# NethermindEth/zinc

Measured on AMD Instinct MI355X. Metric: Zip commit+open MCoeffs/s at 2^24 witness, higher is better.
Workload: dtype i64

## Files before the change

### include/zip_hip.h

```cpp
#ifndef ZIP_HIP_H
#define ZIP_HIP_H

#include <stddef.h>
#include <stdint.h>

#ifdef __cplusplus
extern "C" {
#endif

#define ZIP_HIP_ABI_VERSION 3

#define ZIP_OK 0
#define ZIP_ERR_INVALID_PARAM (-1)
#define ZIP_ERR_SHAPE (-2)
#define ZIP_ERR_HIP (-3)
#define ZIP_ERR_NO_DEVICE (-4)
#define ZIP_ERR_UNSUPPORTED (-5)
#define ZIP_ERR_ALLOC (-6)
#define ZIP_ERR_NULL (-7)

typedef enum { ZIP_MEM_HOST = 0, ZIP_MEM_DEVICE = 1 } zip_mem_kind;

typedef struct zip_ctx zip_ctx;
typedef struct zip_commitment zip_commitment;
// ... 35 lines not shown
int32_t zip_commit(zip_ctx *ctx, const int64_t *evals, size_t n_evals, zip_mem_kind evals_kind,
                   int32_t with_merkle, uint8_t *roots_out, zip_commitment **out);
void zip_commitment_free(zip_commitment *c);

int32_t zip_ctx_set_speculation(zip_ctx *ctx, int32_t on);

int32_t zip_commit_hinted(zip_ctx *ctx, const int64_t *evals, size_t n_evals, zip_mem_kind evals_kind,
                          const uint32_t *cols, uint32_t n_cols, uint8_t *roots_out, zip_commitment **out);

int32_t zip_commitment_device_ptrs(zip_commitment *c, uint64_t **rows, uint8_t **layers, uint8_t **roots);
int32_t zip_commit_download(zip_commitment *c, uint64_t *rows_out, uint8_t *layers_out, uint8_t *roots_out);
int32_t zip_commitment_upload(zip_ctx *ctx, const uint64_t *rows, const uint8_t *layers, const uint8_t *roots,
                              zip_commitment **out);


int32_t zip_open_testing(zip_ctx *ctx, const int64_t *evals, zip_mem_kind evals_kind, const int64_t *coeffs,
                         uint64_t *uprime_out, zip_mem_kind out_kind);
int32_t zip_open_columns(zip_commitment *c, const uint32_t *cols, uint32_t n_cols, uint8_t *wire_out,
                         zip_mem_kind out_kind);
int32_t zip_open_eval(zip_ctx *ctx, const int64_t *evals, zip_mem_kind evals_kind, const uint64_t *q0_mont,
                      const zip_field *field, uint64_t *row_out, zip_mem_kind out_kind);
size_t zip_proof_len(const zip_ctx *ctx, uint32_t n_cols, uint32_t field_limbs);
int32_t zip_open(zip_commitment *c, const int64_t *evals, zip_mem_kind evals_kind, const int64_t *coeffs,
                 const uint32_t *cols, uint32_t n_cols, const uint64_t *q0_mont, const zip_field *field,
                 uint8_t *proof_out, zip_mem_kind out_kind);

int32_t zip_open_shard(zip_commitment *c, const int64_t *evals_d, const int64_t *coeffs, const uint32_t *cols, uint32_t n_cols,
                       const uint64_t *q0_mont, const zip_field *field, uint64_t *uprime_part_d, uint64_t *row_part_d,
                       uint8_t *wire_d);

int32_t zip_commit_open(zip_ctx *ctx, const int64_t *evals, size_t n_evals, zip_mem_kind evals_kind, const int64_t *coeffs,
                        const uint32_t *cols, uint32_t n_cols, const uint64_t *q0_mont, const zip_field *field,
                        uint8_t *roots_out, uint8_t *proof_out, zip_mem_kind out_kind, zip_commitment **out);

typedef struct zip_job zip_job;
int32_t zip_commit_open_begin(zip_ctx *ctx, const int64_t *evals_d, size_t n_evals, const int64_t *coeffs,
                              const uint32_t *cols, uint32_t n_cols, const uint64_t *q0_mont, const zip_field *field,
                              uint8_t *proof_out_d, zip_job **job);
int32_t zip_job_wait(zip_job *job, uint8_t *roots_out);

typedef struct zip_batch zip_batch;
int32_t zip_batch_commit(zip_ctx *ctx, const int64_t *evals, size_t n_evals, uint32_t n_polys, zip_mem_kind evals_kind,
                         uint8_t *roots_out, zip_batch **out);
uint32_t zip_batch_size(const zip_batch *b);
void zip_batch_free(zip_batch *b);
int32_t zip_batch_member(zip_batch *b, uint32_t index, zip_commitment **out);
int32_t zip_batch_open_eval(zip_batch *b, const uint64_t *q0_mont, const zip_field *field, uint64_t *rows_out,
                            zip_mem_kind out_kind);
int32_t zip_batch_open(zip_batch *b, const int64_t *coeffs, const uint32_t *cols, uint32_t n_cols, const uint64_t *q0_mont,
                       const zip_field *field, uint8_t *proofs_out, zip_mem_kind out_kind);

typedef int32_t (*zip_proof_sink)(void *user, const uint8_t *bytes, size_t len);
int32_t zip_open_stream(zip_commitment *c, const int64_t *evals, zip_mem_kind evals_kind, const int64_t *coeffs,
                        const uint32_t *cols, uint32_t n_cols, const uint64_t *q0_mont, const zip_field *field,
                        zip_proof_sink sink, void *user, size_t chunk_bytes);

typedef enum {
    ZIP_VERIFY_ACCEPT = 0,
    ZIP_VERIFY_PROXIMITY_TESTING = 1,
    ZIP_VERIFY_EVAL_CONSISTENCY = 2,
    ZIP_VERIFY_PROXIMITY_Q0 = 3,
    ZIP_VERIFY_MERKLE = 4,
    ZIP_VERIFY_MALFORMED = 5,
    ZIP_VERIFY_OVERFLOW = 6
} zip_verify_verdict;
typedef struct {
    int32_t verdict;
    uint32_t column;
    uint32_t bad_merkle_paths;
    uint32_t malformed_paths;
} zip_verify_report;
int32_t zip_verify(zip_ctx *ctx, const uint8_t *roots, const uint8_t *proof, zip_mem_kind proof_kind, size_t proof_len,
                   const int64_t *coeffs, const uint32_t *cols, uint32_t n_cols, const uint64_t *q0_mont,
                   const uint64_t *q1_mont, const uint64_t *eval_mont, const zip_field *field,
                   zip_verify_report *report);

typedef struct zip_sumcheck zip_sumcheck;
typedef struct {
    uint32_t n_terms;
    uint32_t term_mask[8];
    uint64_t coeff[8][8];
} zip_sumcheck_comb;
int32_t zip_sumcheck_init(int32_t device, const uint64_t *const *mles, zip_mem_kind kind, uint32_t n_mles,
                          uint32_t num_vars, uint32_t degree, const zip_sumcheck_comb *comb, const zip_field *field,
                          zip_sumcheck **out);
int32_t zip_sumcheck_round(zip_sumcheck *s, const uint64_t *r_prev, uint64_t *evaluations_out);
int32_t zip_sumcheck_round_begin(zip_sumcheck *s, const uint64_t *r_prev);
int32_t zip_sumcheck_round_end(zip_sumcheck *s, uint64_t *evaluations_out);
const char *zip_sumcheck_last_error(const zip_sumcheck *s);
void zip_sumcheck_free(zip_sumcheck *s);

typedef struct {
    uint64_t st[25];
    uint8_t buf[136];
    uint32_t buflen;
} zip_keccak_state;

int32_t zip_sumcheck_prove(zip_sumcheck *s, zip_keccak_state *transcript, uint64_t *msgs_out, uint64_t *randomness_out);
void zip_sumcheck_launch_counts(uint64_t *round_kernel_rounds, uint64_t *tail_kernel_launches);

typedef struct zip_ccs zip_ccs;
typedef struct {
    uint32_t n_rows, n_cols;
    const uint32_t *row_ptr, *col_idx;
    const int64_t *values;
} zip_sparse_matrix;
typedef enum { ZIP_CCS_Z_FIELD = 0, ZIP_CCS_MZ = 1, ZIP_CCS_EQ = 2, ZIP_CCS_SECOND = 3 } zip_ccs_table_kind;
int32_t zip_ccs_create(int32_t device, const zip_sparse_matrix *matrices, uint32_t t, uint32_t s, const zip_field *field,
                       zip_ccs **out);
void zip_ccs_free(zip_ccs *c);
const char *zip_ccs_last_error(const zip_ccs *c);
int32_t zip_ccs_set_z(zip_ccs *c, const int64_t *z, size_t z_len, zip_mem_kind kind);
int32_t zip_ccs_eq_table(zip_ccs *c, const uint64_t *r, uint32_t slot);
int32_t zip_ccs_second_table(zip_ccs *c, const uint64_t *r_x, const uint64_t *gamma, uint64_t *v_s_out);
int32_t zip_ccs_eval_matrices(zip_ccs *c, const uint64_t *r_x, const uint64_t *r_y, uint64_t *v_xy_out);
int32_t zip_ccs_table(zip_ccs *c, zip_ccs_table_kind which, uint32_t index, const uint64_t **table_dev);
int32_t zip_ccs_download(zip_ccs *c, zip_ccs_table_kind which, uint32_t index, uint64_t *out);

int32_t zip_field_map_int256(zip_ctx *ctx, const uint64_t *values, uint32_t n, const zip_field *field, uint64_t *out);

int32_t zip_mle_eval(zip_ctx *ctx, const int64_t *evals, zip_mem_kind evals_kind, const uint64_t *q0_mont,
                     const uint64_t *q1_mont, const zip_field *field, uint64_t *value_out);
int32_t zip_commitment_mle_eval(zip_commitment *c, const uint64_t *q0_mont, const uint64_t *q1_mont,
                                const zip_field *field, uint64_t *value_out);

int32_t zip_sum_partials(zip_ctx *ctx, const uint64_t *uparts, const uint64_t *fparts, uint32_t n_parts,
                         const zip_field *field, uint64_t *uprime_out, uint64_t *row_out);

typedef struct zip_mctx zip_mctx;
int32_t zip_mctx_create(const zip_params *params, int32_t n_devices, const int32_t *devices, zip_mctx **out);
void zip_mctx_destroy(zip_mctx *m);
const char *zip_mctx_last_error(const zip_mctx *m);
uint32_t zip_mctx_shards(const zip_mctx *m);
zip_ctx *zip_mctx_shard_ctx(zip_mctx *m, uint32_t shard);
int32_t zip_mctx_set_witness(zip_mctx *m, const int64_t *evals, size_t n_evals);
int32_t zip_mctx_commit_open(zip_mctx *m, const int64_t *evals, const int64_t *coeffs, const uint32_t *cols,
                             uint32_t n_cols, const uint64_t *q0_mont, const zip_field *field, uint8_t *roots_out,
                             uint8_t *proof_out);
int32_t zip_mctx_shard_openings(zip_mctx *m, uint32_t shard, uint8_t **ptr, size_t *bytes, uint32_t *row_begin,
                                uint32_t *row_count);
int32_t zip_mctx_ends(zip_mctx *m, uint8_t **ptr, size_t *u_bytes, size_t *row_bytes);
int32_t zip_mctx_roots(zip_mctx *m, uint32_t shard, uint8_t **ptr);
const char *zip_mctx_roots_path(const zip_mctx *m);

int32_t zip_merkle_trees(int32_t device, const uint64_t *leaves, uint32_t leaf_limbs, uint32_t depth,
                         uint32_t num_trees, zip_mem_kind kind, uint8_t *layers_out);

typedef struct {
    const char *name;
    uint32_t launches;
    float total_ms;
} zip_kernel_time;
int32_t zip_ctx_set_profiling(zip_ctx *ctx, int32_t on);
int32_t zip_ctx_commit_clock(zip_ctx *ctx, double *mhz_out);
int32_t zip_ctx_profile_read(zip_ctx *ctx, zip_kernel_time *out, uint32_t cap);

#ifdef __cplusplus
}
#endif
#endif
```

### zinc_amd/cabi.py

```python
import ctypes as C
import os

import numpy as np

_PKG = os.path.dirname(os.path.abspath(__file__))
LIB_PATH = os.environ.get("ZIP_HIP_LIB_PATH") or os.path.join(_PKG, "lib", "libzip_hip.so")

ZIP_OK = 0
ZIP_ERR_INVALID_PARAM = -1
ZIP_ERR_SHAPE = -2
ZIP_ERR_HIP = -3
ZIP_ERR_NO_DEVICE = -4
ZIP_ERR_UNSUPPORTED = -5
ZIP_ERR_ALLOC = -6
ZIP_ERR_NULL = -7
MEM_HOST, MEM_DEVICE = 0, 1

EXPORTED_SYMBOLS = (
    "zip_abi_version", "zip_strerror", "zip_device_count", "zip_release_cached_memory", "zip_host_register", "zip_host_unregister", "zip_ctx_create", "zip_ctx_destroy",
    "zip_ctx_last_error", "zip_ctx_synchronize", "zip_ctx_stream", "zip_ctx_set_speculation", "zip_commit", "zip_commit_hinted", "zip_commit_open", "zip_commit_open_begin", "zip_job_wait", "zip_commitment_free",
    "zip_commitment_device_ptrs", "zip_commit_download", "zip_commitment_upload", "zip_open_testing",
    "zip_open_columns", "zip_open_eval", "zip_proof_len", "zip_open", "zip_open_shard", "zip_sum_partials", "zip_merkle_trees",
    "zip_ctx_set_profiling", "zip_ctx_profile_read", "zip_ctx_commit_clock",
    "zip_mctx_create", "zip_mctx_destroy", "zip_mctx_last_error", "zip_mctx_shards", "zip_mctx_shard_ctx", "zip_mctx_set_witness",
    "zip_mctx_commit_open", "zip_mctx_shard_openings", "zip_mctx_ends", "zip_mctx_roots", "zip_mctx_roots_path", "zip_verify", "zip_mle_eval", "zip_commitment_mle_eval", "zip_field_map_int256",
    "zip_open_stream", "zip_sumcheck_init", "zip_sumcheck_round", "zip_sumcheck_round_begin", "zip_sumcheck_round_end", "zip_sumcheck_last_error", "zip_sumcheck_free",
    "zip_sumcheck_prove", "zip_sumcheck_launch_counts",
    "zip_ccs_create", "zip_ccs_free", "zip_ccs_last_error", "zip_ccs_set_z", "zip_ccs_eq_table",
    "zip_ccs_second_table", "zip_ccs_table", "zip_ccs_download", "zip_ccs_eval_matrices",
    "zip_batch_commit", "zip_batch_size", "zip_batch_free", "zip_batch_member", "zip_batch_open_eval", "zip_batch_open",
)


class Job:

    def __init__(self, ctx, handle, keep):
        self._ctx, self._h, self._keep = ctx, handle, keep

    def wait(self, want_roots=False):
        assert self._h is not None, "job already waited for"
        roots = np.zeros((self._ctx.rows_local, 32), dtype=np.uint8) if want_roots else None
        h, self._h = self._h, None
        rc = lib().zip_job_wait(h, roots.ctypes.data if roots is not None else None)
        self._keep = None
        self._ctx._check(rc, "zip_job_wait")
        return roots

    def close(self):
        if self._h is not None:
            h, self._h = self._h, None
            try:
                lib().zip_job_wait(h, None)
            finally:
                self._keep = None

    def __enter__(self):
        return self

    def __exit__(self, *exc):
        self.close()

    def __del__(self):
        try:
            self.close()
        except Exception:
            pass


class ZipError(RuntimeError):
    def __init__(self, code, what, detail=""):
        self.code = code
        super().__init__(f"{what}: {strerror(code)} ({code})" + (f": {detail}" if detail else ""))


class ZipParams(C.Structure):
    _fields_ = [
        ("num_vars", C.c_uint32), ("row_len", C.c_uint32), ("num_rows", C.c_uint32),
        ("codeword_len", C.c_uint32), ("rep", C.c_uint32),
        ("n_limbs", C.c_uint32), ("k_limbs", C.c_uint32), ("m_limbs", C.c_uint32),
        ("perm1", C.POINTER(C.c_uint32)), ("perm2", C.POINTER(C.c_uint32)),
        ("device", C.c_int32), ("row_begin", C.c_uint32), ("row_count", C.c_uint32),
    ]


class ZipField(C.Structure):
    _fields_ = [("limbs", C.c_uint32), ("modulus", C.c_uint64 * 8)]


class VerifyReport(C.Structure):
    _fields_ = [("verdict", C.c_int32), ("column", C.c_uint32), ("bad_merkle_paths", C.c_uint32),
                ("malformed_paths", C.c_uint32)]


VERIFY_ACCEPT, VERIFY_PROXIMITY_TESTING, VERIFY_EVAL_CONSISTENCY, VERIFY_PROXIMITY_Q0 = 0, 1, 2, 3
VERIFY_MERKLE, VERIFY_MALFORMED, VERIFY_OVERFLOW = 4, 5, 6


class SumcheckComb(C.Structure):
    _fields_ = [("n_terms", C.c_uint32), ("term_mask", C.c_uint32 * 8), ("coeff", (C.c_uint64 * 8) * 8)]


class KeccakState(C.Structure):
    _fields_ = [("st", C.c_uint64 * 25), ("buf", C.c_uint8 * 136), ("buflen", C.c_uint32)]

    @classmethod
    def make(cls, st=None, buf=b""):
        k = cls()
        if st is not None:
            for i, w in enumerate(st):
                k.st[i] = int(w)
        for i, b in enumerate(bytes(buf)):
            k.buf[i] = b
        k.buflen = len(buf)
        return k

    def pending(self) -> bytes:
        return bytes(self.buf[: self.buflen])


def make_comb(term_masks, coeffs_limbs):
    c = SumcheckComb()
    c.n_terms = len(term_masks)
    cl = np.asarray(coeffs_limbs, dtype=np.uint64).reshape(len(term_masks), -1)
    for t, m in enumerate(term_masks):
        c.term_mask[t] = int(m)
        for i in range(cl.shape[1]):
            c.coeff[t][i] = int(cl[t, i])
    return c


class SparseMatrix(C.Structure):
    _fields_ = [("n_rows", C.c_uint32), ("n_cols", C.c_uint32), ("row_ptr", C.c_void_p), ("col_idx", C.c_void_p),
                ("values", C.c_void_p)]


CCS_Z_FIELD, CCS_MZ, CCS_EQ, CCS_SECOND = 0, 1, 2, 3

PROOF_SINK = C.CFUNCTYPE(C.c_int32, C.c_void_p, C.c_void_p, C.c_size_t)


class KernelTime(C.Structure):
    _fields_ = [("name", C.c_char_p), ("launches", C.c_uint32), ("total_ms", C.c_float)]


_lib = None


def lib():
    global _lib
    if _lib is not None:
        return _lib
    try:
        import torch
    except ImportError:
        pass
    if not os.path.exists(LIB_PATH):
        raise RuntimeError(
            f"{LIB_PATH} is missing: build it with `python -m zinc_amd.build` "
            "(__graft_entry__.build()).  The Zip HIP path has no CPU fallback.")
    L = C.CDLL(LIB_PATH)
    vp, u8p, u32p, u64p, i64p = C.c_void_p, C.c_void_p, C.c_void_p, C.c_void_p, C.c_void_p
    L.zip_abi_version.restype = C.c_int32
    L.zip_strerror.restype = C.c_char_p
    L.zip_strerror.argtypes = [C.c_int32]
    L.zip_device_count.restype = C.c_int32
    L.zip_release_cached_memory.restype = None
    L.zip_host_register.argtypes = [C.c_void_p, C.c_size_t]
    L.zip_host_unregister.argtypes = [C.c_void_p]
    L.zip_host_unregister.restype = None
    L.zip_ctx_create.argtypes = [C.POINTER(ZipParams), C.POINTER(vp)]
    L.zip_ctx_destroy.argtypes = [vp]
    L.zip_ctx_destroy.restype = None
    L.zip_ctx_last_error.argtypes = [vp]
    L.zip_ctx_last_error.restype = C.c_char_p
    L.zip_ctx_synchronize.argtypes = [vp]
    L.zip_ctx_stream.argtypes = [vp]
    L.zip_ctx_stream.restype = vp
    L.zip_commit.argtypes = [vp, i64p, C.c_size_t, C.c_int, C.c_int32, u8p, C.POINTER(vp)]
    L.zip_commit_hinted.argtypes = [vp, i64p, C.c_size_t, C.c_int, u32p, C.c_uint32, u8p, C.POINTER(vp)]
    L.zip_commit_open.argtypes = [vp, i64p, C.c_size_t, C.c_int, i64p, u32p, C.c_uint32, u64p, C.POINTER(ZipField), u8p, vp,
                                  C.c_int, C.POINTER(vp)]
    L.zip_commit_open.restype = C.c_int32
    L.zip_commit_open_begin.argtypes = [vp, i64p, C.c_size_t, i64p, u32p, C.c_uint32, u64p, C.POINTER(ZipField), vp, C.POINTER(vp)]
    L.zip_commit_open_begin.restype = C.c_int32
    L.zip_job_wait.argtypes = [vp, u8p]
    L.zip_job_wait.restype = C.c_int32
    L.zip_verify.argtypes = [vp, u8p, vp, C.c_int, C.c_size_t, i64p, u32p, C.c_uint32, u64p, u64p, u64p,
                             C.POINTER(ZipField), C.POINTER(VerifyReport)]
    L.zip_mle_eval.argtypes = [vp, i64p, C.c_int, u64p, u64p, C.POINTER(ZipField), u64p]
    L.zip_commitment_mle_eval.argtypes = [vp, u64p, u64p, C.POINTER(ZipField), u64p]
    L.zip_field_map_int256.argtypes = [vp, u64p, C.c_uint32, C.POINTER(ZipField), u64p]
    L.zip_open_stream.argtypes = [vp, i64p, C.c_int, i64p, u32p, C.c_uint32, u64p, C.POINTER(ZipField), PROOF_SINK,
                                  vp, C.c_size_t]
    L.zip_sumcheck_init.argtypes = [C.c_int32, vp, C.c_int, C.c_uint32, C.c_uint32, C.c_uint32, C.POINTER(SumcheckComb),
                                    C.POINTER(ZipField), C.POINTER(vp)]
    L.zip_sumcheck_round.argtypes = [vp, u64p, u64p]
    L.zip_sumcheck_round_begin.argtypes = [vp, u64p]
    L.zip_sumcheck_round_end.argtypes = [vp, u64p]
    L.zip_sumcheck_prove.argtypes = [vp, C.POINTER(KeccakState), u64p, u64p]
    L.zip_sumcheck_launch_counts.argtypes = [C.POINTER(C.c_uint64), C.POINTER(C.c_uint64)]
    L.zip_sumcheck_launch_counts.restype = None
    L.zip_sumcheck_last_error.argtypes = [vp]
    L.zip_sumcheck_last_error.restype = C.c_char_p
    L.zip_sumcheck_free.argtypes = [vp]
    L.zip_sumcheck_free.restype = None
    L.zip_ccs_create.argtypes = [C.c_int32, C.POINTER(SparseMatrix), C.c_uint32, C.c_uint32, C.POINTER(ZipField),
                                 C.POINTER(vp)]
    L.zip_ccs_free.argtypes = [vp]
    L.zip_ccs_free.restype = None
    L.zip_ccs_last_error.argtypes = [vp]
    L.zip_ccs_last_error.restype = C.c_char_p
    L.zip_ccs_set_z.argtypes = [vp, i64p, C.c_size_t, C.c_int]
    L.zip_ccs_eq_table.argtypes = [vp, u64p, C.c_uint32]
    L.zip_ccs_second_table.argtypes = [vp, u64p, u64p, u64p]
    L.zip_ccs_table.argtypes = [vp, C.c_int, C.c_uint32, C.POINTER(vp)]
    L.zip_ccs_eval_matrices.argtypes = [vp, u64p, u64p, u64p]
    L.zip_ccs_download.argtypes = [vp, C.c_int, C.c_uint32, u64p]
    L.zip_commitment_free.argtypes = [vp]
    L.zip_commitment_free.restype = None
    L.zip_batch_commit.argtypes = [vp, i64p, C.c_size_t, C.c_uint32, C.c_int, u8p, C.POINTER(vp)]
    L.zip_batch_size.argtypes = [vp]
    L.zip_batch_size.restype = C.c_uint32
    L.zip_batch_free.argtypes = [vp]
    L.zip_batch_free.restype = None
    L.zip_batch_member.argtypes = [vp, C.c_uint32, C.POINTER(vp)]
    L.zip_batch_open_eval.argtypes = [vp, u64p, C.POINTER(ZipField), u64p, C.c_int]
    L.zip_batch_open.argtypes = [vp, i64p, u32p, C.c_uint32, u64p, C.POINTER(ZipField), u8p, C.c_int]
    for fn in ("zip_batch_commit", "zip_batch_member", "zip_batch_open_eval", "zip_batch_open"):
        getattr(L, fn).restype = C.c_int32
    L.zip_commitment_device_ptrs.argtypes = [vp, C.POINTER(vp), C.POINTER(vp), C.POINTER(vp)]
    L.zip_commit_download.argtypes = [vp, u64p, u8p, u8p]
    L.zip_commitment_upload.argtypes = [vp, u64p, u8p, u8p, C.POINTER(vp)]
    L.zip_open_testing.argtypes = [vp, i64p, C.c_int, i64p, u64p, C.c_int]
    L.zip_open_columns.argtypes = [vp, u32p, C.c_uint32, u8p, C.c_int]
    L.zip_open_eval.argtypes = [vp, i64p, C.c_int, u64p, C.POINTER(ZipField), u64p, C.c_int]
    L.zip_proof_len.argtypes = [vp, C.c_uint32, C.c_uint32]
    L.zip_proof_len.restype = C.c_size_t
    L.zip_open.argtypes = [vp, i64p, C.c_int, i64p, u32p, C.c_uint32, u64p, C.POINTER(ZipField), u8p, C.c_int]
    L.zip_open_shard.argtypes = [vp, i64p, i64p, u32p, C.c_uint32, u64p, C.POINTER(ZipField), u64p, u64p, u8p]
    L.zip_open_shard.restype = C.c_int32
    L.zip_sum_partials.argtypes = [vp, u64p, u64p, C.c_uint32, C.POINTER(ZipField), u64p, u64p]
    L.zip_merkle_trees.argtypes = [C.c_int32, u64p, C.c_uint32, C.c_uint32, C.c_uint32, C.c_int, u8p]
    L.zip_ctx_set_profiling.argtypes = [vp, C.c_int32]
    L.zip_ctx_profile_read.argtypes = [vp, C.POINTER(KernelTime), C.c_uint32]
    L.zip_ctx_commit_clock.argtypes = [vp, C.POINTER(C.c_double)]
    L.zip_ctx_commit_clock.restype = C.c_int32
    L.zip_mctx_create.argtypes = [C.POINTER(ZipParams), C.c_int32, C.POINTER(C.c_int32), C.POINTER(vp)]
    L.zip_mctx_destroy.argtypes = [vp]
    L.zip_mctx_destroy.restype = None
    L.zip_mctx_last_error.argtypes = [vp]
    L.zip_mctx_last_error.restype = C.c_char_p
    L.zip_mctx_shards.argtypes = [vp]
    L.zip_mctx_shards.restype = C.c_uint32
    L.zip_mctx_shard_ctx.argtypes = [vp, C.c_uint32]
    L.zip_mctx_shard_ctx.restype = vp
    L.zip_mctx_set_witness.argtypes = [vp, i64p, C.c_size_t]
    L.zip_mctx_commit_open.argtypes = [vp, i64p, i64p, u32p, C.c_uint32, u64p, C.POINTER(ZipField), u8p, u8p]
    L.zip_mctx_shard_openings.argtypes = [vp, C.c_uint32, C.POINTER(vp), C.POINTER(C.c_size_t), C.POINTER(C.c_uint32),
                                          C.POINTER(C.c_uint32)]
    L.zip_mctx_ends.argtypes = [vp, C.POINTER(vp), C.POINTER(C.c_size_t), C.POINTER(C.c_size_t)]
    L.zip_mctx_roots.argtypes = [vp, C.c_uint32, C.POINTER(vp)]
    L.zip_mctx_roots.restype = C.c_int32
    L.zip_mctx_roots_path.argtypes = [vp]
    L.zip_mctx_roots_path.restype = C.c_char_p
    for fn in ("zip_mctx_create", "zip_mctx_set_witness", "zip_mctx_commit_open", "zip_mctx_shard_openings", "zip_mctx_ends"):
        getattr(L, fn).restype = C.c_int32
    for fn in ("zip_ctx_create", "zip_ctx_synchronize", "zip_commit", "zip_commit_hinted", "zip_commitment_device_ptrs",
               "zip_commit_download", "zip_commitment_upload", "zip_open_testing", "zip_open_columns",
               "zip_open_eval", "zip_open", "zip_sum_partials", "zip_merkle_trees", "zip_ctx_set_profiling",
               "zip_ctx_profile_read", "zip_verify", "zip_mle_eval", "zip_field_map_int256", "zip_open_stream", "zip_sumcheck_init", "zip_sumcheck_round"):
        getattr(L, fn).restype = C.c_int32
    _lib = L
    return L


def strerror(code):
    return lib().zip_strerror(code).decode()


def device_count():
    return lib().zip_device_count()


def make_field(modulus: int, limbs: int) -> ZipField:
    f = ZipField()
    f.limbs = limbs
    for i in range(8):
        f.modulus[i] = (modulus >> (64 * i)) & 0xFFFFFFFFFFFFFFFF if i < limbs else 0
    return f


def _ptr(x):
    if x is None:
        return None, MEM_HOST
    if isinstance(x, np.ndarray):
        assert x.flags["C_CONTIGUOUS"]
        return x.ctypes.data, MEM_HOST
    if hasattr(x, "data_ptr"):
        assert x.is_contiguous()
        return x.data_ptr(), (MEM_DEVICE if x.is_cuda else MEM_HOST)
    raise TypeError(type(x))


def geometry(num_vars, rep=2):
    n = 1 << num_vars
    isqrt = int(np.floor(np.sqrt(n)))
    while isqrt * isqrt > n:
        isqrt -= 1
    while (isqrt + 1) * (isqrt + 1) <= n:
        isqrt += 1
    row_len = 1
    while row_len < isqrt:
        row_len <<= 1
    num_rows = 1
    while num_rows < n // row_len:
        num_rows <<= 1
    return row_len, num_rows, row_len * rep


class ZipContext:

    def __init__(self, num_vars, perm1, perm2, device=0, rep=2, row_begin=0, row_count=0,
                 n_limbs=1, k_limbs=4, m_limbs=8, geometry_override=None):
        L = lib()
        row_len, num_rows, cw = geometry_override or geometry(num_vars, rep)
        self.num_vars, self.row_len, self.num_rows, self.codeword_len, self.rep = num_vars, row_len, num_rows, cw, rep
        self.depth = max(cw - 1, 0).bit_length() if cw > 1 else 0
        self.rows_local = row_count or num_rows
        self.row_begin = row_begin
        self.k_limbs, self.m_limbs = k_limbs, m_limbs
        self._perm1 = np.ascontiguousarray(perm1, dtype=np.uint32)
        self._perm2 = np.ascontiguousarray(perm2, dtype=np.uint32)
        p = ZipParams(num_vars, row_len, num_rows, cw, rep, n_limbs, k_limbs, m_limbs,
                      self._perm1.ctypes.data_as(C.POINTER(C.c_uint32)),
                      self._perm2.ctypes.data_as(C.POINTER(C.c_uint32)), device, row_begin, row_count)
        h = C.c_void_p()
        rc = L.zip_ctx_create(C.byref(p), C.byref(h))
        if rc != ZIP_OK:
            raise ZipError(rc, "zip_ctx_create")
        self._h = h
        self.device = device

    def close(self):
        if getattr(self, "_h", None):
            lib().zip_ctx_destroy(self._h)
            self._h = None

    def __del__(self):
        try:
            self.close()
        except Exception:
            pass

    def _check(self, rc, what):
        if rc != ZIP_OK:
            raise ZipError(rc, what, lib().zip_ctx_last_error(self._h).decode())

    def synchronize(self):
        self._check(lib().zip_ctx_synchronize(self._h), "zip_ctx_synchronize")

    @property
    def stream(self):
        return lib().zip_ctx_stream(self._h)

    def commit(self, evals, with_merkle=True, want_roots=True, hint_cols=None):
        ptr, kind = _ptr(evals)
        n = evals.size if isinstance(evals, np.ndarray) else evals.numel()
        roots = np.zeros((self.rows_local, 32), dtype=np.uint8) if (with_merkle and want_roots) else None
        h = C.c_void_p()
        rp = roots.ctypes.data if roots is not None else None
        if hint_cols is not None:
            assert with_merkle, "a hint only makes sense for a commitment that will be opened"
            hc = np.ascontiguousarray(hint_cols, dtype=np.uint32)
            rc = lib().zip_commit_hinted(self._h, ptr, n, kind, hc.ctypes.data, hc.size, rp, C.byref(h))
            self._check(rc, "zip_commit_hinted")
        else:
            rc = lib().zip_commit(self._h, ptr, n, kind, int(with_merkle), rp, C.byref(h))
            self._check(rc, "zip_commit")
        return Commitment(self, h, bool(with_merkle)), roots

    def batch_commit(self, evals_2d, want_roots=True):
        ptr, kind = _ptr(evals_2d)
        n = evals_2d.size if isinstance(evals_2d, np.ndarray) else evals_2d.numel()
        n_polys = evals_2d.shape[0] if len(evals_2d.shape) > 1 else 1
        roots = np.zeros((n_polys, self.num_rows, 32), dtype=np.uint8) if want_roots else None
        h = C.c_void_p()
        rc = lib().zip_batch_commit(self._h, ptr, n, n_polys, kind, roots.ctypes.data if roots is not None else None, C.byref(h))
        self._check(rc, "zip_batch_commit")
        return Batch(self, h, evals_2d if kind == MEM_DEVICE else None, roots)

    def commit_open(self, evals, coeffs, cols, q0_mont, field, out=None, want_roots=True, keep=False):
        ptr, kind = _ptr(evals)
        n = evals.size if isinstance(evals, np.ndarray) else evals.numel()
        cols = np.ascontiguousarray(cols, dtype=np.uint32)
        coeffs_c = np.ascontiguousarray(coeffs, dtype=np.int64) if coeffs is not None else None
        q0 = np.ascontiguousarray(q0_mont, dtype=np.uint64) if q0_mont is not None else None
        roots = np.zeros((self.rows_local, 32), dtype=np.uint8) if want_roots else None
        res = out if out is not None else np.zeros(self.proof_len(cols.size, field.limbs), dtype=np.uint8)
        optr, okind = _ptr(res)
# ... 495 lines not shown
```

### zinc_amd/csrc/kernels_commit.cuh

```cuda
#pragma once
#include <hip/hip_runtime.h>
#include <stdint.h>

#include "blake3.cuh"

namespace zipk {

typedef __int128 i128;
typedef unsigned __int128 u128;

#ifdef ZIPK_DEBUG_STAMPS
constexpr uint32_t kStampRec = 64;
__device__ __forceinline__ unsigned long long stamp_hw_id() {
    const uint32_t xcc = __builtin_amdgcn_s_getreg((3 << 11) | 20), hw = __builtin_amdgcn_s_getreg((31 << 11) | 4);
    return (unsigned long long)xcc | ((unsigned long long)hw << 8);
}
#endif

struct CommitArgs {
    const int64_t *evals;
    const uint32_t *perm1;
    const uint32_t *perm2;
    uint64_t *rows;
    uint32_t compact_rows;
    uint32_t *layers;
    uint32_t *roots;
    uint32_t row_len;
    uint32_t cw;
    uint32_t nact;
    uint32_t num_rows;
    uint32_t rounds_per_chunk;
    uint64_t chunk_ends;
    uint8_t *pk;
    uint32_t pk_stride, pk_off0, pk_off1, pk_off2;
    const uint32_t *pk_tab;
    uint32_t *chunk_done;
    uint32_t classes;
    const uint32_t *need;
    unsigned long long *clock;
    uint4 *slab;
#ifdef ZIPK_DEBUG_STAMPS
    unsigned long long *stamps;
#endif
};

__device__ __forceinline__ i128 shfl_up_i96(i128 x, int off) {
    uint32_t d0 = (uint32_t)x, d1 = (uint32_t)((u128)x >> 32), d2 = (uint32_t)((u128)x >> 64);
    d0 = __shfl_up(d0, off, 64);
    d1 = __shfl_up(d1, off, 64);
    d2 = __shfl_up(d2, off, 64);
    const int64_t hi = (int64_t)(int32_t)d2;
    return (i128)(((u128)(uint64_t)hi << 64) | ((u128)d1 << 32) | d0);
}

__device__ __forceinline__ void lds_barrier() {
    asm volatile("s_waitcnt lgkmcnt(0)\n\ts_barrier" ::: "memory");
}

template <int CTRL, int ROW_MASK>
__device__ __forceinline__ i128 dpp_i96(i128 x) {
    const int d0 = (int)(uint32_t)x, d1 = (int)(uint32_t)((u128)x >> 32), d2 = (int)(uint32_t)((u128)x >> 64);
    const uint32_t y0 = (uint32_t)__builtin_amdgcn_update_dpp(0, d0, CTRL, ROW_MASK, 0xF, false);
    const uint32_t y1 = (uint32_t)__builtin_amdgcn_update_dpp(0, d1, CTRL, ROW_MASK, 0xF, false);
    const uint32_t y2 = (uint32_t)__builtin_amdgcn_update_dpp(0, d2, CTRL, ROW_MASK, 0xF, false);
    const int64_t hi = (int64_t)(int32_t)y2;
    return (i128)(((u128)(uint64_t)hi << 64) | ((u128)y1 << 32) | y0);
}

__device__ __forceinline__ i128 block_exclusive_scan_i96(i128 total, i128 *wave_tot, int which) {
    const int lane = threadIdx.x & 63;
    const int wid = __builtin_amdgcn_readfirstlane((int)(threadIdx.x >> 6));
    i128 x = total;
    x += dpp_i96<0x111, 0xF>(x);
    x += dpp_i96<0x112, 0xF>(x);
    x += dpp_i96<0x114, 0xF>(x);
    x += dpp_i96<0x118, 0xF>(x);
    x += dpp_i96<0x142, 0xA>(x);
    x += dpp_i96<0x143, 0xC>(x);
    i128 *tot = wave_tot + 16 * which;
    if (lane == 63) tot[wid] = x;
    lds_barrier();
    i128 t = lane < 16 ? tot[lane] : (i128)0;
    t += dpp_i96<0x111, 0xF>(t);
    t += dpp_i96<0x112, 0xF>(t);
    t += dpp_i96<0x114, 0xF>(t);
    t += dpp_i96<0x118, 0xF>(t);
    i128 base = 0;
    if (wid > 0) {
        const uint32_t b0 = (uint32_t)__builtin_amdgcn_readlane((int)(uint32_t)t, wid - 1);
        const uint32_t b1 = (uint32_t)__builtin_amdgcn_readlane((int)(uint32_t)((u128)t >> 32), wid - 1);
        const uint32_t b2 = (uint32_t)__builtin_amdgcn_readlane((int)(uint32_t)((u128)t >> 64), wid - 1);
        base = (i128)(((u128)(uint64_t)(int64_t)(int32_t)b2 << 64) | ((u128)b1 << 32) | b0);
    }
    return base + (x - total);
}

__device__ __forceinline__ void store_hash(uint32_t *dst, const uint32_t (&h)[8]) {
    uint4 *d = reinterpret_cast<uint4 *>(dst);
    d[0] = make_uint4(h[0], h[1], h[2], h[3]);
    d[1] = make_uint4(h[4], h[5], h[6], h[7]);
}
__device__ __forceinline__ void load_hash(const uint32_t *src, uint32_t (&h)[8]) {
    const uint4 *s = reinterpret_cast<const uint4 *>(src);
    uint4 a = s[0], b = s[1];
    h[0] = a.x; h[1] = a.y; h[2] = a.z; h[3] = a.w;
    h[4] = b.x; h[5] = b.y; h[6] = b.z; h[7] = b.w;
}

__device__ __forceinline__ uint32_t level_off(uint32_t cw, uint32_t k) { return 2u * cw - ((2u * cw) >> k); }

template <bool ILV>
__device__ __forceinline__ uint32_t *tree_of(uint32_t *layers, uint32_t cw, uint32_t row) {
    return ILV ? layers + ((size_t)(row >> 2) * (2u * cw) * 4 + (row & 3u)) * 8 : layers + (size_t)row * (2u * cw) * 8;
}
template <bool ILV>
constexpr uint32_t kNodeWords = ILV ? 32u : 8u;

__device__ __forceinline__ uint32_t round_slot(uint32_t b, uint32_t G, uint32_t classes = 1) {
    if (G & 7u) return b;
    const uint32_t x = b & 7u, l = b >> 3;
    if (classes <= 1u) return x * (G >> 3) + l;
    const uint32_t per = (G >> 3) / classes, k = l / per;
    return k * (G / classes) + x * per + (l - k * per);
}
__device__ __forceinline__ uint32_t commit_class(uint32_t b, uint32_t G, uint32_t classes) {
    return classes <= 1u ? 0u : (b >> 3) / ((G >> 3) / classes);
}

template <int LVL, int E0, class Src>
__device__ __forceinline__ void subtree_hash(Src &src, uint32_t (&h)[8]) {
    if constexpr (LVL == 0) {
        src.template leaf<E0>(h);
    } else {
        uint32_t l[8], r[8];
        subtree_hash<LVL - 1, E0>(src, l);
        subtree_hash<LVL - 1, E0 + (1 << (LVL - 1))>(src, r);
        blake3_node(l, r, h);
        src.store(LVL, E0 >> LVL, h);
    }
}

constexpr int kStoreAll = 0, kStoreHinted = 1, kStorePacked = 3;

template <int E, int MODE = kStoreAll, bool LAZY = false>
struct StridedLeaves {
    static constexpr bool MASKED = MODE != kStoreAll;
    uint32_t w0[E], w1[E], w2[E];
    const uint64_t *lz_lo = nullptr;
    const uint32_t *lz_hi = nullptr;
    uint32_t lz_stride = 0;
    template <int E0>
    __device__ __forceinline__ void entry(uint32_t &a, uint32_t &b, uint32_t &c) const {
        if (LAZY) {
            const uint64_t lo = lz_lo[E0 * lz_stride];
            a = (uint32_t)lo;
            b = (uint32_t)(lo >> 32);
            c = lz_hi[E0 * lz_stride];
        } else {
            a = w0[E0];
            b = w1[E0];
            c = w2[E0];
        }
    }
    uint64_t *out_row;
    uint32_t *tree;
    uint32_t cw, T, tid;
    uint32_t base = 0;
    uint32_t compact = 0;
    uint32_t smask = 0xFFFFFFFFu;
    static constexpr uint32_t NW = MODE == kStorePacked ? 32u : 8u;
    uint8_t *pk_v = nullptr, *pk_n = nullptr;
    uint32_t pk_off0 = 0, pk_off1 = 0, pk_off2 = 0;
    __device__ __forceinline__ void set_packed(const CommitArgs &a, uint32_t row) {
        uint8_t *g = a.pk + (size_t)(row >> 2) * 4 * a.pk_stride;
        pk_v = g + (row & 3u) * 16u;
        pk_n = g + (row & 3u) * 32u;
        pk_off0 = 4u * a.pk_off0;
        pk_off1 = 4u * a.pk_off1;
        pk_off2 = 4u * a.pk_off2;
    }
    uint32_t ptab[16] = {};
    template <int K>
    __device__ __forceinline__ uint32_t pbase() const { return (ptab[K >> 1] >> ((K & 1) * 16)) & 0xFFFFu; }
    static __device__ __forceinline__ uint32_t lanes_below(uint64_t m) {
        return __builtin_amdgcn_mbcnt_hi((uint32_t)(m >> 32), __builtin_amdgcn_mbcnt_lo((uint32_t)m, 0u));
    }
    template <int E0>
    __device__ __forceinline__ void store_row_of(uint32_t d0, uint32_t d1, uint32_t d2) {
        if (MASKED && !(smask & (1u << E0))) return;
        const uint32_t j = base + E0 * T + tid;
        const uint32_t s = (uint32_t)((int32_t)d2 >> 31);
        if (MODE == kStorePacked) {
            const uint32_t pos = pbase<E0>() + lanes_below(__builtin_amdgcn_ballot_w64(true));
            *reinterpret_cast<uint4 *>(pk_v + (size_t)pos * 64) = make_uint4(d0, d1, d2, s);
        } else if (compact) {
            *reinterpret_cast<uint4 *>(out_row + (size_t)j * 2) = make_uint4(d0, d1, d2, s);
        } else {
            uint4 *o = reinterpret_cast<uint4 *>(out_row + (size_t)j * 4);
            o[0] = make_uint4(d0, d1, d2, s);
            o[1] = make_uint4(s, s, s, s);
        }
    }
    template <int E0>
    __device__ __forceinline__ void store_row() {
        uint32_t d0, d1, d2;
        entry<E0>(d0, d1, d2);
        store_row_of<E0>(d0, d1, d2);
    }
    template <int E0>
    __device__ __forceinline__ void leaf(uint32_t (&h)[8]) {
        uint32_t d0, d1, d2;
        entry<E0>(d0, d1, d2);
        store_row_of<E0>(d0, d1, d2);
        blake3_leaf_sext96(d0, d1, d2, h);
        if (!MASKED || (smask & (0x100u << E0))) {
            if (MODE == kStorePacked) {
                const uint32_t pos = pbase<8 + E0>() + lanes_below(__builtin_amdgcn_ballot_w64(true));
                store_hash(reinterpret_cast<uint32_t *>(pk_n + pk_off0) + (size_t)pos * 32, h);
            } else {
                store_hash(tree + (size_t)(base + E0 * T + tid) * 8, h);
            }
        }
    }
    template <int LVL, int E0>
    __device__ __forceinline__ void store(const uint32_t (&h)[8]) {
        if (MASKED && LVL <= 2 && !(smask & ((LVL == 1 ? 0x10000u : 0x1000000u) << (E0 >> LVL)))) return;
        const uint32_t e = E0 + (tid & ((1u << LVL) - 1u));
        const uint32_t n = (base + e * T + tid) >> LVL;
        if (MODE == kStorePacked && LVL == 1) {
            const uint64_t act = __builtin_amdgcn_ballot_w64(true);
            const bool odd = tid & 1u;
            const uint32_t pos = (odd ? pbase<16 + (E0 >> 1) * 2 + 1>() : pbase<16 + (E0 >> 1) * 2>()) +
                                 lanes_below(act & (odd ? 0xAAAAAAAAAAAAAAAAull : 0x5555555555555555ull));
            store_hash(reinterpret_cast<uint32_t *>(pk_n + pk_off1) + (size_t)pos * 32, h);
        } else if (MODE == kStorePacked && LVL == 2) {
            const uint64_t act = __builtin_amdgcn_ballot_w64(true);
            const uint32_t q = tid & 3u;
            constexpr int K0 = 24 + ((E0 >> 2) & 1) * 4;
            const uint32_t b01 = (q & 1u) ? pbase<K0 + 1>() : pbase<K0>(), b23 = (q & 1u) ? pbase<K0 + 3>() : pbase<K0 + 2>();
            const uint32_t pos = ((q & 2u) ? b23 : b01) + lanes_below(act & (0x1111111111111111ull << q));
            store_hash(reinterpret_cast<uint32_t *>(pk_n + pk_off2) + (size_t)pos * 32, h);
        } else {
            store_hash(tree + ((size_t)level_off(cw, LVL) + n) * NW, h);
        }
    }
};

template <int E>
__device__ __forceinline__ uint32_t store_mask(const uint32_t *need, uint32_t cw, uint32_t base, uint32_t T, uint32_t tid) {
    if (!need) return 0xFFFFFFFFu;
    const uint32_t *nv = need, *n0 = nv + (cw + 31) / 32, *n1 = n0 + (cw + 31) / 32, *n2 = n1 + (cw / 2 + 31) / 32;
    uint32_t m = 0;
#pragma unroll
    for (int e = 0; e < E; e++) {
        const uint32_t j = base + e * T + tid;
        m |= ((nv[j >> 5] >> (j & 31)) & 1u) << e;
        m |= ((n0[j >> 5] >> (j & 31)) & 1u) << (8 + e);
    }
#pragma unroll
    for (int g = 0; g < E / 2; g++) {
        const uint32_t i = (base + (2 * g + (tid & 1u)) * T + tid) >> 1;
        m |= ((n1[i >> 5] >> (i & 31)) & 1u) << (16 + g);
    }
#pragma unroll
    for (int g = 0; g < E / 4; g++) {
        const uint32_t i = (base + (4 * g + (tid & 3u)) * T + tid) >> 2;
        m |= ((n2[i >> 5] >> (i & 31)) & 1u) << (24 + g);
    }
    return m;
}

template <int E, int E0, class Src>
__device__ __forceinline__ void store_rows_only(Src &src) {
    if constexpr (E0 < E) {
        src.template store_row<E0>();
        store_rows_only<E, E0 + 1>(src);
    }
}

template <int LVL, int E0, class Src>
__device__ __forceinline__ void bfly_hash(Src &src, uint32_t (&h)[8]) {
    if constexpr (LVL == 0) {
        src.template leaf<E0>(h);
    } else {
        uint32_t A[8], B[8], m[16];
        bfly_hash<LVL - 1, E0>(src, A);
        bfly_hash<LVL - 1, E0 + (1 << (LVL - 1))>(src, B);
        const bool up = (src.tid >> (LVL - 1)) & 1;
#pragma unroll
        for (int i = 0; i < 8; i++) {
            const uint32_t snd = up ? A[i] : B[i];
            const uint32_t rcv = __shfl_xor(snd, 1 << (LVL - 1), 64);
            m[i] = up ? rcv : A[i];
            m[8 + i] = up ? B[i] : rcv;
        }
        blake3_block64(m, h);
        src.template store<LVL, E0>(h);
    }
}

template <bool ILV>
__device__ __forceinline__ void upper_stage(const CommitArgs &a, uint32_t first, uint32_t nrows_c, uint32_t lvl, uint32_t nl,
                                            uint32_t lane, uint32_t nlanes) {
    constexpr uint32_t NW = kNodeWords<ILV>;
    const uint32_t cw = a.cw, depth = 31u - __builtin_clz(cw);
    const uint32_t u_shift = depth - (lvl - 1u) - nl;
    const uint32_t total = nrows_c << u_shift;
    const uint32_t slot0 = round_slot(blockIdx.x, gridDim.x, a.classes);
    for (uint32_t idx = lane; idx < total; idx += nlanes) {
        const uint32_t ri = idx >> u_shift, i = idx & ((1u << u_shift) - 1u);
        const uint32_t r = slot0 + (first + ri) * gridDim.x;
        uint32_t *tree = tree_of<ILV>(a.layers, cw, r);
        const uint32_t *ch = tree + ((size_t)level_off(cw, lvl - 1u) + ((size_t)i << nl)) * NW;
        uint32_t c0[8], c1[8], h0[8];
        load_hash(ch, c0);
        load_hash(ch + NW, c1);
        if (nl == 1u) {
            blake3_node(c0, c1, h0);
            store_hash(tree + ((size_t)level_off(cw, lvl) + i) * NW, h0);
            if (lvl == depth) store_hash(a.roots + (size_t)r * 8, h0);
        } else {
            uint32_t c2[8], c3[8], h1[8], h2[8];
            blake3_node(c0, c1, h0);
            uint32_t *o = tree + ((size_t)level_off(cw, lvl) + 2u * i) * NW;
            store_hash(o, h0);
            asm volatile("" ::: "memory");
            load_hash(ch + 2 * NW, c2);
            load_hash(ch + 3 * NW, c3);
            blake3_node(c2, c3, h1);
            store_hash(o + NW, h1);
            blake3_node(h0, h1, h2);
            store_hash(tree + ((size_t)level_off(cw, lvl + 1u) + i) * NW, h2);
            if (lvl + 1u == depth) store_hash(a.roots + (size_t)r * 8, h2);
        }
    }
}

struct ChunkCursor {
    uint32_t first = 0, index = 0;
    __device__ __forceinline__ bool ends_with(const CommitArgs &a, uint32_t round, bool last) const {
        if (last) return true;
        if (a.chunk_ends) return (a.chunk_ends >> round) & 1u;
        return (round + 1) % a.rounds_per_chunk == 0;
    }
    __device__ __forceinline__ void advance(uint32_t round) {
        first = round + 1;
        index++;
    }
};

constexpr uint32_t kFinisherFlagWords = 16;

template <bool HASH, bool ILV = false>
struct ChunkFinisher {
    bool pending = false;
    uint32_t p_first = 0, p_nrows = 0, p_lvl = 0, p_index = 0;
    uint32_t p_base = 0;
    uint32_t n_deferred = 0;
    uint32_t *flags = nullptr;

    __device__ __forceinline__ void init(uint32_t *lds_flags, uint32_t tid) {
        flags = lds_flags;
        if (tid < kFinisherFlagWords) lds_flags[tid] = 0;
    }

    __device__ __forceinline__ void top_of_row() const {
        if (HASH && pending) asm volatile("s_waitcnt vmcnt(0)" ::: "memory");
    }

    static __device__ __forceinline__ void publish(const CommitArgs &a, uint32_t index, uint32_t lane) {
        if (!a.chunk_done) return;
        asm volatile("s_waitcnt vmcnt(0)" ::: "memory");
        if (lane == 0) {
            __builtin_amdgcn_fence(__ATOMIC_RELEASE, "agent");
            asm volatile("s_waitcnt vmcnt(0)" ::: "memory");
            __hip_atomic_fetch_add(&a.chunk_done[index], 1u, __ATOMIC_RELAXED, __HIP_MEMORY_SCOPE_AGENT);
        }
    }

    static __device__ __forceinline__ void signal(uint32_t *flag, uint32_t lane) {
        asm volatile("s_waitcnt vmcnt(0)" ::: "memory");
        if (lane == 0) __hip_atomic_fetch_add(flag, 1u, __ATOMIC_RELEASE, __HIP_MEMORY_SCOPE_WORKGROUP);
    }
    static __device__ __forceinline__ void wait_for(uint32_t *flag, uint32_t target) {
        uint32_t spins = 0;
        while (__hip_atomic_load(flag, __ATOMIC_ACQUIRE, __HIP_MEMORY_SCOPE_WORKGROUP) < target) {
            __builtin_amdgcn_s_sleep(2);
            if (++spins > (1u << 24)) __builtin_trap();
        }
    }

    static __device__ __forceinline__ bool stage_wide(uint32_t cw, uint32_t lvl, uint32_t nl, uint32_t j) {
        return j == 0u || (cw >> (lvl - 1u + nl)) >= 64u;
    }
    static __device__ __forceinline__ uint32_t stage_waves(uint32_t cw, uint32_t depth, uint32_t lvl0, uint32_t j, uint32_t W) {
        const uint32_t lvl = lvl0 + 2u * j;
        if (lvl > depth) return 0u;
        return stage_wide(cw, lvl, depth - lvl >= 1u ? 2u : 1u, j) ? W : 1u;
    }
    __device__ __forceinline__ uint32_t target(uint32_t cw, uint32_t depth, uint32_t j, uint32_t W) const {
        return (n_deferred - 1u) * stage_waves(cw, depth, p_base, j, W) + stage_waves(cw, depth, p_lvl, j, W);
    }
    __device__ __forceinline__ void after_hash(const CommitArgs &a, uint32_t wave, uint32_t lane, uint32_t T) {
        if (!(HASH && pending)) return;
        pending = false;
        n_deferred++;
        constexpr uint32_t kFinWaves = 8u;
        const uint32_t W = T >= 64u * kFinWaves ? kFinWaves : T >= 256u ? 4u : (T + 63u) / 64u;
        if (wave >= W) return;
        const uint32_t cw = a.cw, depth = 31u - __builtin_clz(cw);
        uint32_t lvl = p_lvl, j = 0, owner = 0;
        bool wide = true;
        while (lvl <= depth) {
            const uint32_t nl = depth - lvl >= 1u ? 2u : 1u;
            wide = stage_wide(cw, lvl, nl, j);
            if (wide) {
                if (j) wait_for(flags + (j - 1u), target(cw, depth, j - 1u, W));
                upper_stage<ILV>(a, p_first, p_nrows, lvl, nl, lane + 64u * wave, 64u * W);
                signal(flags + j, lane);
            } else {
                owner = j % W;
                if (wave == owner) {
                    wait_for(flags + (j - 1u), target(cw, depth, j - 1u, W));
                    upper_stage<ILV>(a, p_first, p_nrows, lvl, nl, lane, 64u);
                    signal(flags + j, lane);
                }
            }
            lvl += nl;
            j++;
        }
        if (j == 0u || wide) owner = 0u;
        if (wave == owner) {
            if (j && wide) wait_for(flags + (j - 1u), target(cw, depth, j - 1u, W));
            publish(a, p_index, lane);
        }
    }

    __device__ __forceinline__ void after_loop(const CommitArgs &a, uint32_t wave, uint32_t lane, uint32_t T, unsigned char *lds,
                                               uint32_t lds_bytes) {
        if (!(HASH && pending)) return;
        __syncthreads();
        const uint32_t cw = a.cw, depth = 31u - __builtin_clz(cw);
        const uint32_t tid = lane + 64u * wave;
        const uint32_t w_in0 = cw >> (p_lvl - 1u);
        const uint32_t n_in0 = p_nrows * w_in0;
        if (p_lvl <= depth && (n_in0 + n_in0 / 2u) * 32u <= lds_bytes && n_in0 >= 2u) {
            constexpr uint32_t NW = kNodeWords<ILV>;
            pending = false;
            uint4 *bufA = reinterpret_cast<uint4 *>(lds), *bufB = bufA + 2u * n_in0;
            const uint32_t slot0 = round_slot(blockIdx.x, gridDim.x, a.classes);
            const uint32_t sh0 = 31u - __builtin_clz(w_in0);
            for (uint32_t idx = tid; idx < n_in0; idx += T) {
                const uint32_t ri = idx >> sh0, i = idx & (w_in0 - 1u);
                const uint32_t r = slot0 + (p_first + ri) * gridDim.x;
                const uint4 *src = reinterpret_cast<const uint4 *>(tree_of<ILV>(a.layers, cw, r) + ((size_t)level_off(cw, p_lvl - 1u) + i) * NW);
                bufA[2u * idx] = src[0];
                bufA[2u * idx + 1u] = src[1];
            }
            __syncthreads();
            uint4 *in = bufA, *out = bufB;
            for (uint32_t lvl = p_lvl; lvl <= depth; lvl++) {
                const uint32_t w = cw >> lvl, sh = 31u - __builtin_clz(w), m = p_nrows * w;
                for (uint32_t idx = tid; idx < m; idx += T) {
                    const uint32_t ri = idx >> sh, i = idx & (w - 1u);
                    const uint32_t r = slot0 + (p_first + ri) * gridDim.x;
                    const uint4 a0 = in[4u * idx], a1 = in[4u * idx + 1u], b0 = in[4u * idx + 2u], b1 = in[4u * idx + 3u];
                    const uint32_t c0[8] = {a0.x, a0.y, a0.z, a0.w, a1.x, a1.y, a1.z, a1.w};
                    const uint32_t c1[8] = {b0.x, b0.y, b0.z, b0.w, b1.x, b1.y, b1.z, b1.w};
                    uint32_t h[8];
                    blake3_node(c0, c1, h);
                    store_hash(tree_of<ILV>(a.layers, cw, r) + ((size_t)level_off(cw, lvl) + i) * NW, h);
                    if (lvl == depth) store_hash(a.roots + (size_t)r * 8, h);
                    out[2u * idx] = make_uint4(h[0], h[1], h[2], h[3]);
                    out[2u * idx + 1u] = make_uint4(h[4], h[5], h[6], h[7]);
                }
                __syncthreads();
                uint4 *t = in;
                in = out;
                out = t;
            }
            if (wave == 0u) publish(a, p_index, lane);
            return;
        }
        after_hash(a, wave, lane, T);
    }

    __device__ __forceinline__ void chunk_end(const CommitArgs &a, uint32_t first_level, const ChunkCursor &cc, uint32_t round,
                                              bool last, uint32_t tid, uint32_t T) {
        const uint32_t wave = __builtin_amdgcn_readfirstlane(tid >> 6), lane = tid & 63u;
        if (!HASH) {
            if (a.chunk_done) {
                __syncthreads();
                if (wave == 0) publish(a, cc.index, lane);
            }
            return;
        }
        const uint32_t cw = a.cw, depth = 31u - __builtin_clz(cw);
        const uint32_t first = cc.first, nrows_c = round - first + 1;
        uint32_t lvl = first_level;
        const bool now = last || lvl > depth;
        if (now) {
            __syncthreads();
            if (lvl <= depth) {
                const uint32_t nl = depth - lvl >= 1u ? 2u : 1u;
                upper_stage<ILV>(a, first, nrows_c, lvl, nl, tid, T);
                lvl += nl;
            }
        }
        if (depth == 0 && tid == 0) {
            for (uint32_t ri = 0; ri < nrows_c; ri++) {
                const uint32_t r = round_slot(blockIdx.x, gridDim.x, a.classes) + (first + ri) * gridDim.x;
                uint32_t h[8];
                load_hash(a.layers + (size_t)r * (2u * cw) * 8, h);
                store_hash(a.roots + (size_t)r * 8, h);
            }
        }
        if (!last) p_base = lvl;
        pending = true;
        p_first = first;
        p_nrows = nrows_c;
        p_lvl = lvl;
        p_index = cc.index;
    }
};

__device__ __forceinline__ void stamp_clock(const CommitArgs &a, int slot) {
    if (a.clock && blockIdx.x == 0 && threadIdx.x == 0) {
        a.clock[2 * slot] = __builtin_amdgcn_s_memtime();
        a.clock[2 * slot + 1] = __builtin_amdgcn_s_memrealtime();
    }
}

__device__ __forceinline__ uint32_t opaque_zero(uint32_t dep) {
    uint32_t z;
    asm volatile("s_mov_b32 %0, 0" : "=s"(z) : "s"(dep));
    return z;
}

template <int E, bool HASH, int MODE = kStoreAll>
__global__ void __launch_bounds__(1024, 4) raa_commit_kernel(CommitArgs a) {
    constexpr bool MASKED = MODE != kStoreAll;
    extern __shared__ __align__(16) unsigned char smem[];
    constexpr int LOGE = (E == 1) ? 0 : (E == 2) ? 1 : (E == 4) ? 2 : 3;
    static_assert((1 << LOGE) == E && E <= 8, "E must be 1, 2, 4 or 8");

    const uint32_t tid0 = threadIdx.x, T = blockDim.x;
    constexpr uint32_t PAD = 32 / E;
    const uint32_t PS = T + PAD;
    const uint32_t cw = a.cw, row_len = a.row_len;
    const bool active = tid0 < a.nact;
    stamp_clock(a, 0);

    i128 *wave_tot = reinterpret_cast<i128 *>(smem);
    uint64_t *t2lo = reinterpret_cast<uint64_t *>(smem + 512);
    uint32_t *t2hi = reinterpret_cast<uint32_t *>(t2lo + E * PS);
    int64_t *rowbuf = reinterpret_cast<int64_t *>(t2hi + E * PS);
    uint32_t pidx[E];
    auto load_pidx = [&](uint32_t t) {
#pragma unroll
        for (int e = 0; e < E; e++) {
            uint32_t v1 = 0, v2 = 0;
            if (active) {
                v1 = a.perm1[t * E + e] & (row_len - 1);
                const uint32_t p2 = a.perm2[t * E + e];
                v2 = (p2 & (E - 1)) * PS + (p2 >> LOGE);
            }
            pidx[e] = v1 | (v2 << 16);
        }
    };
    load_pidx(tid0);
    const uint32_t smask = (MASKED && active) ? store_mask<E>(a.need, cw, 0u, a.nact, tid0) : 0xFFFFFFFFu;
    uint32_t ptab[16] = {};
    if (MODE == kStorePacked) {
        const uint32_t *wt = a.pk_tab + (size_t)__builtin_amdgcn_readfirstlane(tid0 >> 6) * 16;
#pragma unroll
        for (int k = 0; k < 16; k++) ptab[k] = __builtin_amdgcn_readfirstlane(wt[k]);
    }
    constexpr int NPF = (E >= 2) ? E / 2 : 1;
    const bool prefetch = row_len == NPF * T;
    int64_t nxt[NPF];

#ifdef ZIPK_DEBUG_STAMPS
    unsigned long long ph_a = 0, ph_b = 0, ph_c = 0, ph_t;
    if (tid0 == 0 && a.stamps) {
        a.stamps[(size_t)kStampRec * blockIdx.x] = wall_clock64();
        a.stamps[(size_t)kStampRec * blockIdx.x + 2] = stamp_hw_id();
    }
#define ZIPK_PH(acc) do { const unsigned long long now_ = wall_clock64(); acc += now_ - ph_t; ph_t = now_; } while (0)
#else
#define ZIPK_PH(acc) do { } while (0)
#endif
    uint32_t round = 0;
    ChunkCursor cc;
    if (a.classes > 1u) {
        const uint32_t c = commit_class(blockIdx.x, gridDim.x, a.classes);
        cc.index = c;
        const uint32_t prio = (a.classes - 1u - c) * 3u / (a.classes - 1u);
        if (prio == 3u) __builtin_amdgcn_s_setprio(3);
        else if (prio == 2u) __builtin_amdgcn_s_setprio(2);
        else if (prio == 1u) __builtin_amdgcn_s_setprio(1);
    }
    ChunkFinisher<HASH, MODE == kStorePacked> fin;
    fin.init(reinterpret_cast<uint32_t *>(rowbuf + row_len), tid0);
    const uint32_t wave0 = __builtin_amdgcn_readfirstlane(tid0 >> 6);
    for (uint32_t row = round_slot(blockIdx.x, gridDim.x, a.classes); row < a.num_rows; row += gridDim.x, round++) {
#ifdef ZIPK_DEBUG_STAMPS
        ph_t = wall_clock64();
#endif
        const uint32_t z = opaque_zero(row);
        const uint32_t tid = tid0 + z;
        const int64_t *in = a.evals + (size_t)row * row_len;
        uint64_t *out_row = a.rows + (size_t)row * cw * (a.compact_rows ? 2 : 4);

        const bool has_next = row + gridDim.x < a.num_rows;
        if (!(prefetch && round)) {
            if (round) lds_barrier();
            for (uint32_t i = tid; i < row_len; i += T) rowbuf[i] = in[i];
            lds_barrier();
        }
        if (prefetch && has_next) {
            const int64_t *nin = a.evals + (size_t)(row + gridDim.x) * row_len;
#pragma unroll
            for (int k = 0; k < NPF; k++) nxt[k] = nin[k * T + tid];
        }

        i128 v[E];
        if (active) {
#pragma unroll
            for (int e = 0; e < E; e++) v[e] = (i128)rowbuf[(pidx[e] ^ z) & 0xFFFFu];
#pragma unroll
            for (int e = 1; e < E; e++) v[e] += v[e - 1];
        } else {
#pragma unroll
            for (int e = 0; e < E; e++) v[e] = 0;
        }
        {
            const i128 pre = block_exclusive_scan_i96(v[E - 1], wave_tot, 0);
            if (active) {
#pragma unroll
                for (int e = 0; e < E; e++) {
                    v[e] += pre;
                    const uint32_t slot = e * PS + tid;
                    t2lo[slot] = (uint64_t)v[e];
                    t2hi[slot] = (uint32_t)((u128)v[e] >> 64);
                }
            }
        }
        lds_barrier();
        if (active) {
#pragma unroll
            for (int e = 0; e < E; e++) {
                const uint32_t slot = (pidx[e] ^ z) >> 16;
                const uint64_t lo = t2lo[slot];
                const int64_t hi = (int64_t)(int32_t)t2hi[slot];
                v[e] = (i128)(((u128)(uint64_t)hi << 64) | lo);
            }
#pragma unroll
            for (int e = 1; e < E; e++) v[e] += v[e - 1];
        }
        {
            const i128 pre = block_exclusive_scan_i96(v[E - 1], wave_tot, 1);
#pragma unroll
            for (int e = 0; e < E; e++) v[e] += pre;
        }

        if (active) {
#pragma unroll
            for (int e = 0; e < E; e++) {
                const uint32_t slot = e * PS + tid;
                t2lo[slot] = (uint64_t)v[e];
                t2hi[slot] = (uint32_t)((u128)v[e] >> 64);
            }
        }
        if (prefetch && has_next) {
#pragma unroll
            for (int k = 0; k < NPF; k++) rowbuf[k * T + tid] = nxt[k];
        }
        fin.top_of_row();
        lds_barrier();
        ZIPK_PH(ph_a);
        if (active) {
            StridedLeaves<E, MODE, true> src;
            src.out_row = out_row;
            src.compact = a.compact_rows;
            src.tree = HASH ? tree_of<MODE == kStorePacked>(a.layers, cw, row) : nullptr;
            src.cw = cw;
            src.T = a.nact;
            src.tid = tid;
            src.smask = smask;
            if (MODE == kStorePacked) {
                src.set_packed(a, row);
#pragma unroll
                for (int k = 0; k < 16; k++) src.ptab[k] = ptab[k];
            }
            {
                const uint32_t slot0 = (tid & (E - 1)) * PS + (tid >> LOGE);
                src.lz_lo = t2lo + slot0;
                src.lz_hi = t2hi + slot0;
                src.lz_stride = a.nact >> LOGE;
            }
            if (HASH) {
                uint32_t top[8];
                bfly_hash<LOGE, 0>(src, top);
            } else {
                store_rows_only<E, 0>(src);
            }
        }
        ZIPK_PH(ph_b);
        fin.after_hash(a, wave0, tid0 & 63u, T);
        const bool last = row + gridDim.x >= a.num_rows;
        if (cc.ends_with(a, round, last)) {
            fin.chunk_end(a, LOGE + 1, cc, round, last, tid, T);
            cc.advance(round);
        }
        ZIPK_PH(ph_c);
#ifdef ZIPK_DEBUG_STAMPS
        if (tid0 == 0 && a.stamps && round < kStampRec - 8) a.stamps[(size_t)kStampRec * blockIdx.x + 8 + round] = ph_t;
#endif
    }
    fin.after_loop(a, wave0, tid0 & 63u, T, smem + 512, (uint32_t)(E * PS * 12u));
    stamp_clock(a, 1);
#ifdef ZIPK_DEBUG_STAMPS
    if (tid0 == 0 && a.stamps) {
        unsigned long long *o = a.stamps + (size_t)kStampRec * blockIdx.x;
        o[1] = wall_clock64();
        o[3] = ph_a; o[4] = ph_b; o[5] = ph_c; o[6] = round;
    }
#endif
}

constexpr size_t c16_lds_bytes(uint32_t T) {
    return 512 + (size_t)16 * (T + 2) * 8 + (size_t)16 * (T + 2) + (size_t)T * 4 + 64;
}

template <int B, int P = 0>
__device__ __forceinline__ void transpose8_stage(uint32_t (&x)[8], bool up) {
    if constexpr (P < 4) {
        constexpr int r = ((P >> B) << (B + 1)) | (P & ((1 << B) - 1)), r2 = r | (1 << B);
        const uint32_t lo = x[r], hi = x[r2];
        const uint32_t rcv = __shfl_xor(up ? lo : hi, 1 << B, 64);
        x[r] = up ? rcv : lo;
        x[r2] = up ? hi : rcv;
        transpose8_stage<B, P + 1>(x, up);
    }
}
__device__ __forceinline__ void transpose8(uint32_t (&x)[8], uint32_t lane) {
    transpose8_stage<0>(x, lane & 1u);
    transpose8_stage<1>(x, (lane >> 1) & 1u);
    transpose8_stage<2>(x, (lane >> 2) & 1u);
}

template <uint32_t T, bool HASH, int MODE = kStoreAll>
__global__ void __launch_bounds__(T, 4) raa_commit16_kernel(CommitArgs a) {
    constexpr bool MASKED = MODE != kStoreAll;
    static_assert(MODE == kStoreAll || MODE == kStoreHinted || MODE == kStorePacked, "store mode");
    extern __shared__ __align__(16) unsigned char smem[];
    constexpr int E = 16;
    constexpr uint32_t PS = T + 2;
    const uint32_t tid0 = threadIdx.x;
    const uint32_t cw = a.cw, row_len = a.row_len;
    stamp_clock(a, 0);

    i128 *wave_tot = reinterpret_cast<i128 *>(smem);
    uint64_t *t2lo = reinterpret_cast<uint64_t *>(smem + 512);
    int8_t *t2dh = reinterpret_cast<int8_t *>(t2lo + (size_t)E * PS);
    int32_t *ghi = reinterpret_cast<int32_t *>(t2dh + (size_t)E * PS);
    uint64_t *park_lo = reinterpret_cast<uint64_t *>(smem + 512);
    uint32_t *park_hi = reinterpret_cast<uint32_t *>(park_lo + (size_t)8 * PS);

    const uint32_t smask0 = MASKED ? store_mask<8>(a.need, cw, 0u, 16u, (tid0 & ~7u) * 16u + (tid0 & 7u)) : 0xFFFFFFFFu;
    const uint32_t smask1 = MASKED ? store_mask<8>(a.need, cw, 0u, 16u, (tid0 & ~7u) * 16u + 8u + (tid0 & 7u)) : 0xFFFFFFFFu;
    uint32_t ptab0[16] = {}, ptab1[16] = {};
    if (MODE == kStorePacked) {
        const uint32_t *wt = a.pk_tab + (size_t)__builtin_amdgcn_readfirstlane(tid0 >> 6) * 32;
#pragma unroll
        for (int k = 0; k < 16; k++) {
            ptab0[k] = __builtin_amdgcn_readfirstlane(wt[k]);
            ptab1[k] = __builtin_amdgcn_readfirstlane(wt[16 + k]);
        }
    }

    uint32_t round = 0;
    ChunkCursor cc;
    ChunkFinisher<HASH, MODE == kStorePacked> fin;
    fin.init(reinterpret_cast<uint32_t *>(ghi + T), tid0);
    const uint32_t wave0 = __builtin_amdgcn_readfirstlane(tid0 >> 6);
    for (uint32_t row = round_slot(blockIdx.x, gridDim.x, a.classes); row < a.num_rows; row += gridDim.x, round++) {
        fin.top_of_row();
        const uint32_t z = opaque_zero(row);
        const uint32_t tid = tid0 + z;
        const int64_t *in = a.evals + (size_t)row * row_len;
        uint64_t *out_row = a.rows + (size_t)row * cw * (a.compact_rows ? 2 : 4);

        uint32_t p2[E];
        i128 v[E];
        {
            const uint4 *q1 = reinterpret_cast<const uint4 *>(a.perm1 + (size_t)tid * E);
            const uint4 *q2 = reinterpret_cast<const uint4 *>(a.perm2 + (size_t)tid * E);
#pragma unroll
            for (int k = 0; k < E / 4; k++) {
                const uint4 s1 = q1[k], s2 = q2[k];
                v[4 * k + 0] = (i128)in[s1.x & (row_len - 1)];
                v[4 * k + 1] = (i128)in[s1.y & (row_len - 1)];
                v[4 * k + 2] = (i128)in[s1.z & (row_len - 1)];
                v[4 * k + 3] = (i128)in[s1.w & (row_len - 1)];
                p2[4 * k + 0] = s2.x;
                p2[4 * k + 1] = s2.y;
                p2[4 * k + 2] = s2.z;
                p2[4 * k + 3] = s2.w;
            }
        }
#pragma unroll
        for (int e = 1; e < E; e++) v[e] += v[e - 1];
        {
            const i128 pre = block_exclusive_scan_i96(v[E - 1], wave_tot, 0);
            const int32_t phi = (int32_t)(uint32_t)((u128)pre >> 64);
            ghi[tid] = phi;
#pragma unroll
            for (int e = 0; e < E; e++) {
                const i128 t = v[e] + pre;
                t2lo[e * PS + tid] = (uint64_t)t;
                t2dh[e * PS + tid] = (int8_t)((int32_t)(uint32_t)((u128)t >> 64) - phi);
            }
        }
        lds_barrier();
#pragma unroll
        for (int e = 0; e < E; e++) {
            const uint32_t j = p2[e];
            const uint32_t slot = (j & 15u) * PS + (j >> 4);
            const uint64_t lo = t2lo[slot];
            const int64_t hi = (int64_t)(ghi[j >> 4] + (int32_t)t2dh[slot]);
            v[e] = (i128)(((u128)(uint64_t)hi << 64) | lo);
        }
#pragma unroll
        for (int e = 1; e < E; e++) v[e] += v[e - 1];
        {
            const i128 pre = block_exclusive_scan_i96(v[E - 1], wave_tot, 1);
#pragma unroll
            for (int e = 0; e < E; e++) v[e] += pre;
        }
#pragma unroll
        for (int e = 8; e < E; e++) {
            park_lo[(e - 8) * PS + tid] = (uint64_t)v[e];
            park_hi[(e - 8) * PS + tid] = (uint32_t)((u128)v[e] >> 64);
        }
        uint32_t x0[8], x1[8], x2[8];
#pragma unroll
        for (int e = 0; e < 8; e++) {
            x0[e] = (uint32_t)(uint64_t)v[e];
            x1[e] = (uint32_t)((uint64_t)v[e] >> 32);
            x2[e] = (uint32_t)((u128)v[e] >> 64);
        }
#pragma unroll
        for (uint32_t q = 0; q < 2; q++) {
            if (q) {
#pragma unroll
                for (int e = 0; e < 8; e++) {
                    const uint64_t lo = park_lo[e * PS + tid];
                    x0[e] = (uint32_t)lo;
                    x1[e] = (uint32_t)(lo >> 32);
                    x2[e] = park_hi[e * PS + tid];
                }
            }
            transpose8(x0, tid);
            transpose8(x1, tid);
            transpose8(x2, tid);
            StridedLeaves<8, MODE> src;
            if (MODE == kStorePacked) {
                src.set_packed(a, row);
#pragma unroll
                for (int k = 0; k < 16; k++) src.ptab[k] = q ? ptab1[k] : ptab0[k];
            }
            src.out_row = out_row;
            src.compact = a.compact_rows;
            src.tree = HASH ? tree_of<MODE == kStorePacked>(a.layers, cw, row) : nullptr;
            src.cw = cw;
            src.T = 16;
            src.tid = (tid & ~7u) * 16u + q * 8u + (tid & 7u);
            src.smask = q ? smask1 : smask0;
#pragma unroll
            for (int e = 0; e < 8; e++) {
                src.w0[e] = x0[e];
                src.w1[e] = x1[e];
                src.w2[e] = x2[e];
            }
            if (HASH) {
                uint32_t top[8];
                bfly_hash<3, 0>(src, top);
            } else {
                store_rows_only<8, 0>(src);
            }
        }
        fin.after_hash(a, wave0, tid0 & 63u, T);
        const bool last = row + gridDim.x >= a.num_rows;
        if (cc.ends_with(a, round, last)) {
            fin.chunk_end(a, 4u, cc, round, last, tid, T);
            cc.advance(round);
        }
    }
    fin.after_loop(a, wave0, tid0 & 63u, T, smem + 512, (uint32_t)(E * PS * 9u));
    stamp_clock(a, 1);
}

constexpr uint32_t kSlabThreads = 1024;
constexpr size_t cslab_lds_bytes() {
    return 512 + (size_t)kSlabThreads * 32 + 4 * kFinisherFlagWords;
}

__device__ __forceinline__ void vmem_barrier() {
    asm volatile("s_waitcnt vmcnt(0)" ::: "memory");
    __syncthreads();
}

__device__ __forceinline__ i128 slab_get(const uint4 &u) {
    const int64_t hi = (int64_t)(int32_t)u.z;
    return (i128)(((u128)(uint64_t)hi << 64) | ((u128)u.y << 32) | u.x);
}

template <int E, bool HASH>
__global__ void __launch_bounds__(kSlabThreads, 4) raa_commit_slab_kernel(CommitArgs a) {
    constexpr uint32_t T = kSlabThreads;
    constexpr int LOGE = (E == 32) ? 5 : 6;
    static_assert((1 << LOGE) == E, "E must be 32 or 64");
    extern __shared__ __align__(16) unsigned char smem[];
    const uint32_t tid0 = threadIdx.x;
    const uint32_t cw = a.cw, row_len = a.row_len;
    stamp_clock(a, 0);

    i128 *wave_tot = reinterpret_cast<i128 *>(smem);
    i128 *pre1 = reinterpret_cast<i128 *>(smem + 512);
    i128 *runp = pre1 + T;
    uint4 *slab = a.slab + (size_t)blockIdx.x * cw;

    uint32_t round = 0;
    ChunkCursor cc;
    ChunkFinisher<HASH> fin;
    fin.init(reinterpret_cast<uint32_t *>(runp + T), tid0);
    const uint32_t wave0 = __builtin_amdgcn_readfirstlane(tid0 >> 6);
    for (uint32_t row = round_slot(blockIdx.x, gridDim.x, a.classes); row < a.num_rows; row += gridDim.x, round++) {
        const uint32_t z = opaque_zero(row);
        const uint32_t tid = tid0 + z;
        const int64_t *in = a.evals + (size_t)row * row_len;
        if (round) __syncthreads();

        i128 s = 0;
        {
            const uint4 *q1 = reinterpret_cast<const uint4 *>(a.perm1 + (size_t)tid * E);
#pragma unroll 2
            for (int k = 0; k < E / 4; k++) {
                const uint4 p = q1[k];
                const uint32_t idx[4] = {p.x, p.y, p.z, p.w};
#pragma unroll
                for (int i = 0; i < 4; i++) {
                    s += (i128)in[idx[i] & (row_len - 1)];
                    const u128 u = (u128)s;
                    slab[(size_t)(4 * k + i) * T + tid] = make_uint4((uint32_t)u, (uint32_t)(u >> 32), (uint32_t)(u >> 64), 0u);
                }
            }
        }
        pre1[tid] = block_exclusive_scan_i96(s, wave_tot, 0);
        vmem_barrier();

        const uint4 *q2 = reinterpret_cast<const uint4 *>(a.perm2 + (size_t)tid * E);
        s = 0;
#pragma unroll 2
        for (int k = 0; k < E / 4; k++) {
            const uint4 p = q2[k];
            const uint32_t idx[4] = {p.x, p.y, p.z, p.w};
#pragma unroll
            for (int i = 0; i < 4; i++) {
                const uint32_t j = idx[i];
                s += slab_get(slab[(size_t)(j & (E - 1)) * T + (j >> LOGE)]) + pre1[j >> LOGE];
            }
        }
        runp[tid] = block_exclusive_scan_i96(s, wave_tot, 1);

#pragma unroll 1
        for (uint32_t q = 0; q < (uint32_t)E / 8u; q++) {
            const uint32_t tq = tid + opaque_zero(q);
            uint32_t x0[8], x1[8], x2[8];
            {
                i128 run = runp[tq];
                const uint4 *q2q = reinterpret_cast<const uint4 *>(a.perm2 + (size_t)tq * E) + 2 * q;
                const uint4 pa = q2q[0], pb = q2q[1];
                const uint32_t idx[8] = {pa.x, pa.y, pa.z, pa.w, pb.x, pb.y, pb.z, pb.w};
#pragma unroll
                for (int e = 0; e < 8; e++) {
                    const uint32_t j = idx[e];
                    run += slab_get(slab[(size_t)(j & (E - 1)) * T + (j >> LOGE)]) + pre1[j >> LOGE];
                    const u128 u = (u128)run;
                    x0[e] = (uint32_t)u;
                    x1[e] = (uint32_t)(u >> 32);
                    x2[e] = (uint32_t)(u >> 64);
                }
                runp[tq] = run;
            }
            transpose8(x0, tq);
            transpose8(x1, tq);
            transpose8(x2, tq);
            StridedLeaves<8> src;
            src.out_row = a.rows + (size_t)row * cw * (a.compact_rows ? 2 : 4);
            src.compact = a.compact_rows;
            src.tree = HASH ? tree_of<false>(a.layers, cw, row) : nullptr;
            src.cw = cw;
            src.T = E;
            src.tid = (tq & ~7u) * (uint32_t)E + q * 8u + (tq & 7u);
#pragma unroll
            for (int e = 0; e < 8; e++) {
                src.w0[e] = x0[e];
                src.w1[e] = x1[e];
                src.w2[e] = x2[e];
            }
            if (HASH) {
                uint32_t top[8];
                bfly_hash<3, 0>(src, top);
            } else {
                store_rows_only<8, 0>(src);
            }
        }
        fin.after_hash(a, wave0, tid0 & 63u, T);
        const bool last = row + gridDim.x >= a.num_rows;
        if (cc.ends_with(a, round, last)) {
            fin.chunk_end(a, 4u, cc, round, last, tid, T);
            cc.advance(round);
        }
    }
    fin.after_loop(a, wave0, tid0 & 63u, T, smem + 512, (uint32_t)(T * 32u));
    stamp_clock(a, 1);
}

__global__ void __launch_bounds__(256) witness_digest_kernel(const uint64_t *w, uint64_t n, unsigned long long *out) {
    unsigned long long a = 0, b = 0;
    const uint64_t n2 = n / 2, stride = (uint64_t)gridDim.x * blockDim.x;
    const ulonglong2 *w2 = reinterpret_cast<const ulonglong2 *>(w);
    uint64_t i = (uint64_t)blockIdx.x * blockDim.x + threadIdx.x;
    for (; i + 3 * stride < n2; i += 4 * stride) {
        ulonglong2 v[4];
#pragma unroll
        for (int k = 0; k < 4; k++) v[k] = w2[i + k * stride];
#pragma unroll
        for (int k = 0; k < 4; k++) {
            const uint64_t j = 2 * (i + k * stride);
            a += v[k].x + v[k].y;
            b += v[k].x * (2ull * j + 1ull) + v[k].y * (2ull * j + 3ull);
        }
    }
    for (; i < n2; i += stride) {
        const ulonglong2 v = w2[i];
        a += v.x + v.y;
        b += v.x * (4ull * i + 1ull) + v.y * (4ull * i + 3ull);
    }
    if ((n & 1) && blockIdx.x == 0 && threadIdx.x == 0) {
        a += w[n - 1];
        b += w[n - 1] * (2ull * (n - 1) + 1ull);
    }
    for (int off = 32; off > 0; off >>= 1) {
        a += __shfl_down(a, off, 64);
        b += __shfl_down(b, off, 64);
    }
    if ((threadIdx.x & 63) == 0) {
        atomicAdd(out, a);
        atomicAdd(out + 1, b);
    }
}

__global__ void __launch_bounds__(256) expand_rows_kernel(const uint4 *in, uint4 *out, uint64_t n) {
    for (uint64_t i = (uint64_t)blockIdx.x * blockDim.x + threadIdx.x; i < n; i += (uint64_t)gridDim.x * blockDim.x) {
        const uint4 v = in[i];
        out[2 * i] = v;
        out[2 * i + 1] = make_uint4(v.w, v.w, v.w, v.w);
    }
}

__global__ void __launch_bounds__(64) wait_counter_kernel(uint32_t *counter, uint32_t target, uint32_t zero,
                                                          uint32_t *timeout_flag, unsigned long long timeout_ticks) {
    __builtin_amdgcn_s_setprio(3);
    if (threadIdx.x == 0) {
        const unsigned long long t0 = wall_clock64();
        while (__hip_atomic_fetch_add(counter, zero, __ATOMIC_RELAXED, __HIP_MEMORY_SCOPE_AGENT) < target) {
            __builtin_amdgcn_s_sleep(64);
            if (wall_clock64() - t0 > timeout_ticks) {
                __hip_atomic_store(timeout_flag, 1u, __ATOMIC_RELAXED, __HIP_MEMORY_SCOPE_SYSTEM);
                break;
            }
        }
        __builtin_amdgcn_fence(__ATOMIC_ACQUIRE, "agent");
    }
}

struct UpperNodes {
    const uint32_t *in;
    uint32_t *tree, *root;
    uint32_t cw, level_in, depth, n0;
    template <int E0>
    __device__ __forceinline__ void leaf(uint32_t (&h)[8]) {
        load_hash(in + (size_t)E0 * 8, h);
    }
    __device__ __forceinline__ void store(int lvl, uint32_t idx, const uint32_t (&h)[8]) {
        const uint32_t lv = level_in + lvl;
        store_hash(tree + ((size_t)level_off(cw, lv) + (n0 >> lvl) + idx) * 8, h);
        if (lv == depth) store_hash(root, h);
    }
};

template <int NL>
__global__ void __launch_bounds__(256) merkle_upper_kernel(uint32_t *layers, uint32_t *roots,
                                                           uint32_t num_rows, uint32_t cw,
                                                           uint32_t level_in, uint32_t depth) {
    const uint32_t width_in = cw >> level_in;
    const uint32_t groups = width_in >> NL;
    const uint32_t log_groups = 31u - __builtin_clz(groups);
    const uint32_t gid = blockIdx.x * blockDim.x + threadIdx.x;
    if (gid >= num_rows * groups) return;
    const uint32_t r = gid >> log_groups, g = gid & (groups - 1);
    uint32_t *tree = layers + (size_t)r * (2u * cw) * 8;
    const uint32_t *src_nodes = tree + ((size_t)level_off(cw, level_in) + ((size_t)g << NL)) * 8;
    UpperNodes src{src_nodes, tree, roots + (size_t)r * 8, cw, level_in, depth, g << NL};
    uint32_t top[8];
    subtree_hash<NL, 0>(src, top);
}

__global__ void copy_roots_depth0_kernel(const uint32_t *layers, uint32_t *roots, uint32_t num_rows,
                                         uint32_t cw) {
    const uint32_t r = blockIdx.x * blockDim.x + threadIdx.x;
    if (r >= num_rows) return;
    const uint32_t *tree = layers + (size_t)r * (2u * cw) * 8;
#pragma unroll
    for (int i = 0; i < 8; i++) roots[(size_t)r * 8 + i] = tree[i];
// ... 18 lines not shown
```

### zinc_amd/csrc/zip_hip.hip

```cpp
#include <hip/hip_runtime.h>
#include <dlfcn.h>
#include <algorithm>
#include <atomic>
#include <chrono>
#include <thread>

#include <climits>
#include <cstdarg>
#include <cstdio>
#include <cstdlib>
#include <cstring>
#include <functional>
#include <map>
#include <memory>
#include <mutex>
#include <new>
#include <string>
#include <vector>

#include "../../include/zip_hip.h"
#include "kernels_commit.cuh"
#include "kernels_open.cuh"
#include "kernels_batch.cuh"
#include "kernels_verify.cuh"
#include "kernels_sumcheck.cuh"
#include "kernels_sumcheck_tail.cuh"
#include "kernels_sumcheck_wide.cuh"
#include "kernels_spartan.cuh"
#include "rccl_dyn.h"

using namespace zipk;

namespace {

typedef unsigned __int128 u128;

bool is_pow2(uint64_t x) { return x && !(x & (x - 1)); }
uint32_t ilog2(uint64_t x) { return 63u - (uint32_t)__builtin_clzll(x); }

long env_long(const char *name, long def, long lo, long hi) {
    const char *e = getenv(name);
    if (!e) return def;
    char *end = nullptr;
    const long v = strtol(e, &end, 10);
    return end == e || v < lo || v > hi ? def : v;
}

struct KernelStat {
    uint32_t launches = 0;
    float total_ms = 0.f;
};
struct PendingEvent {
    const char *name;
    hipEvent_t start, stop;
};

}

struct PackedLayout {
    uint32_t stride = 0, off[3] = {};
};
struct HintPlan {
    uint32_t cw = 0, e = 0, threads = 0;
    bool want_packed = false;
    std::vector<uint32_t> cols;
    std::vector<uint32_t> bm;
    bool packed = false;
    PackedLayout L;
    std::vector<uint32_t> wave_tab;
    std::vector<uint16_t> pos[4];
    std::vector<uint16_t> own_ranks;
    unsigned char *dev = nullptr;
    std::function<void(unsigned char *)> release;
    HintPlan() = default;
    HintPlan(const HintPlan &) = delete;
    HintPlan &operator=(const HintPlan &) = delete;
    ~HintPlan() { if (dev && release) release(dev); }
    bool ranks(const uint32_t *cs, uint32_t n, uint16_t *out) const {
        for (uint32_t i = 0; i < n; i++) {
            const uint32_t col = cs[i];
            if (col >= cw) return false;
            const uint16_t r[4] = {pos[0][col], pos[1][col ^ 1u], pos[2][(col >> 1) ^ 1u], pos[3][(col >> 2) ^ 1u]};
            for (int k = 0; k < 4; k++) {
                if (r[k] == 0xFFFF) return false;
                out[4 * i + k] = r[k];
            }
        }
        return true;
    }
};

static inline int speculation_default_flag() {
    const long v = env_long("ZIP_HIP_SPECULATE", -1, 0, 1);
    return v < 0 ? 1 : v == 0 ? 0 : 2;
}

struct zip_ctx {
    zip_params p{};
    uint32_t depth = 0;
    uint32_t rows_local = 0;
    int device = 0;
    hipStream_t stream = nullptr, s_commit = nullptr, s_upper = nullptr;
    uint32_t n_chunks = 1;
    uint32_t knob_rpb = 0;
    int knob_stream = -1;
    std::string knob_chunk_rounds;
    bool no_compact = false;
    uint32_t num_cus = 256;
    uint32_t *timeout_flag_h = nullptr, *timeout_flag_d = nullptr;
    unsigned long long *clock_h = nullptr, *clock_d = nullptr;
    std::vector<hipEvent_t> dep_event_pool;
    uint32_t *perm1_d = nullptr, *perm2_d = nullptr;
    unsigned char *pinned_base = nullptr, *stage_h = nullptr, *stage_big = nullptr;
    size_t stage_cap = 0, stage_big_cap = 0;
    unsigned char *bounce[2] = {nullptr, nullptr};
    size_t bounce_cap = 0;
    std::vector<unsigned char *> hint_free;
    std::shared_ptr<bool> alive = std::make_shared<bool>(true);
    bool profile_commit_only = false;
    std::shared_ptr<HintPlan> hint_plan;
    int speculate = speculation_default_flag();
    bool seen_columns = false;
    uint32_t *ring_d = nullptr;
    uint32_t ring_next = 0, ring_epoch = 0;
    uint4 *slab_d = nullptr;
    size_t slab_bytes = 0;
    unsigned char *job_stage[2] = {nullptr, nullptr};
    size_t job_stage_cap[2] = {0, 0};
    bool job_busy[2] = {false, false};
    uint64_t recover_epoch = 0;
    zip_field field_cache_in{};
    alignas(8) unsigned char field_cache_out[256] = {};
    bool field_cache_valid = false;
    std::string last_error;
    bool recycle = false;
    size_t h2d_bounce_threshold = (size_t)8 << 20;
    std::multimap<size_t, void *> free_blocks;
    std::map<void *, size_t> live_blocks;
    std::mutex mu;
    std::recursive_mutex api_mu;
    bool profiling = false;
    std::vector<PendingEvent> pending;
    std::vector<hipEvent_t> event_pool;
    std::map<std::string, KernelStat> stats;
    std::vector<std::string> stat_names;
};

struct BatchStore {
    void *rows = nullptr, *layers = nullptr, *roots = nullptr, *evals = nullptr;
    std::function<void(BatchStore &)> release;
    BatchStore() = default;
    BatchStore(const BatchStore &) = delete;
    BatchStore &operator=(const BatchStore &) = delete;
    ~BatchStore() { if (release) release(*this); }
};

struct zip_batch {
    zip_ctx *ctx = nullptr;
    uint32_t n_polys = 0;
    std::shared_ptr<BatchStore> store;
    const int64_t *evals_d = nullptr;
};

struct zip_commitment {
    std::shared_ptr<BatchStore> store;
    bool borrows_rows = false, borrows_rest = false;
    const uint32_t *gather_order = nullptr;
    zip_ctx *ctx = nullptr;
    uint64_t *rows = nullptr;
    bool compact_rows = false;
    uint32_t *layers = nullptr;
    uint32_t *roots = nullptr;
    int64_t *evals = nullptr;
    size_t rows_bytes = 0, layers_bytes = 0, roots_bytes = 0, evals_bytes = 0;
    std::vector<uint32_t> bounds, expected;
    uint32_t *chunk_done = nullptr;
    const uint4 *gather_tab = nullptr;
    bool ring_slot = false;
    uint32_t ring_epoch = 0;
    bool consumers_done = false;
    hipEvent_t zeroed = nullptr;
    hipEvent_t done = nullptr;
    std::vector<hipEvent_t> aux;
    bool hinted = false;
    bool packed = false;
    uint32_t pk_stride = 0, pk_off[3] = {};
    std::shared_ptr<HintPlan> plan;
    const uint16_t *rank_d = nullptr;
    std::vector<uint32_t> hint_cols;
    unsigned char *hint_h = nullptr;
    uint32_t *need_d = nullptr;
    const int64_t *evals_ref = nullptr;
    bool speculative = false;
    unsigned long long *digest_d = nullptr;
    hipEvent_t digest_done = nullptr;
    CommitArgs args{};
    uint32_t grid = 0;
};

struct zip_sumcheck {
    zip_ctx *ctx = nullptr;
    uint32_t n_mles = 0, num_vars = 0, degree = 0, fl = 0, round = 0;
    bool pending = false;
    bool proved = false;
    uint64_t *tail_out_d = nullptr;
    const uint64_t *input[kSumcheckMaxMles] = {};
    bool owned = false;
    uint64_t *buf[2][kSumcheckMaxMles] = {};
    uint64_t *partials = nullptr, *evals_d = nullptr;
    uint32_t *done_d = nullptr;
    unsigned char *evals_pinned = nullptr;
    uint32_t max_blocks = 0;
    uint64_t modulus[8] = {};
    uint64_t mont_r[8] = {}, mont_r2[8] = {}, mont_inv = 0;
    uint32_t n_terms = 0, term_mask[8] = {};
    uint64_t coeff[8][8] = {};
};

struct zip_ccs {
    zip_ctx *ctx = nullptr;
    uint32_t t = 0, s = 0, m = 0, fl = 0;
    uint64_t modulus[8] = {};
    struct Mat {
        uint32_t n_rows = 0, nnz = 0;
// ... 425 lines not shown
    uint64_t inv = 0;
    uint64_t quirk_mod = 0;
};
static_assert(sizeof(HostField) <= 256, "zip_ctx::field_cache_out holds a HostField");

int cmp_limbs(const uint64_t *a, const uint64_t *b, uint32_t n) {
    for (uint32_t i = n; i-- > 0;)
        if (a[i] != b[i]) return a[i] < b[i] ? -1 : 1;
    return 0;
}
void sub_limbs(uint64_t *a, const uint64_t *b, uint32_t n) {
    uint64_t borrow = 0;
    for (uint32_t i = 0; i < n; i++) {
        u128 d = (u128)a[i] - b[i] - borrow;
        a[i] = (uint64_t)d;
        borrow = (uint64_t)(d >> 64) & 1;
    }
}
void dbl_mod(uint64_t *x, const uint64_t *q, uint32_t n) {
    const uint64_t top = x[n - 1] >> 63;
    for (uint32_t i = n; i-- > 1;) x[i] = (x[i] << 1) | (x[i - 1] >> 63);
    x[0] <<= 1;
    if (top || cmp_limbs(x, q, n) >= 0) sub_limbs(x, q, n);
}

int32_t make_field_uncached(zip_ctx *ctx, const zip_field *zf, HostField *f);
int32_t make_field(zip_ctx *ctx, const zip_field *zf, HostField *f) {
    if (!zf) return fail(ctx, ZIP_ERR_NULL, "field is NULL");
    if (ctx && ctx->field_cache_valid && ctx->field_cache_in.limbs == zf->limbs &&
        !memcmp(ctx->field_cache_in.modulus, zf->modulus, 8 * (size_t)zf->limbs)) {
        memcpy(f, ctx->field_cache_out, sizeof(HostField));
        return ZIP_OK;
    }
    int32_t rc = make_field_uncached(ctx, zf, f);
    if (!rc && ctx) {
        ctx->field_cache_in = *zf;
        memcpy(ctx->field_cache_out, f, sizeof(HostField));
        ctx->field_cache_valid = true;
    }
    return rc;
}
int32_t make_field_uncached(zip_ctx *ctx, const zip_field *zf, HostField *f) {
    if (!zf) return fail(ctx, ZIP_ERR_NULL, "field is NULL");
    if (zf->limbs < 2 || zf->limbs > 4)
        return fail(ctx, ZIP_ERR_UNSUPPORTED, "field limbs %u not in {2,3,4}", zf->limbs);
    if (!(zf->modulus[0] & 1)) return fail(ctx, ZIP_ERR_INVALID_PARAM, "modulus must be odd");
    const uint32_t n = f->fl = zf->limbs;
    bool gt1 = zf->modulus[0] > 1;
    for (uint32_t i = 1; i < n; i++) gt1 |= zf->modulus[i] != 0;
    if (!gt1) return fail(ctx, ZIP_ERR_INVALID_PARAM, "modulus must be > 1");
    memcpy(f->modulus, zf->modulus, 8 * n);
    uint64_t inv = 1;
    for (int i = 0; i < 63; i++) {
        inv *= inv;
        inv *= f->modulus[0];
    }
    f->inv = (uint64_t)0 - inv;
    uint64_t x[8] = {1};
    for (uint32_t i = 0; i < 64 * n; i++) dbl_mod(x, f->modulus, n);
    memcpy(f->r, x, 8 * n);
    for (uint32_t i = 0; i < 64 * n; i++) dbl_mod(x, f->modulus, n);
    memcpy(f->r2, x, 8 * n);
    f->quirk_mod = 0;
    if (f->modulus[n - 1] >> 63) {
        uint64_t m[8] = {0};
        sub_limbs(m, f->modulus, n);
        bool small = true;
        for (uint32_t i = 1; i < n; i++) small &= (m[i] == 0);
        if (small) f->quirk_mod = m[0];
    }
    return ZIP_OK;
}

template <int FL>
FieldDev<FL> to_dev(const HostField &h) {
    FieldDev<FL> d;
    for (int i = 0; i < FL; i++) {
        d.modulus[i] = h.modulus[i];
        d.r2[i] = h.r2[i];
    }
    d.inv = h.inv;
    return d;
}

int32_t ensure_dynamic_lds(zip_ctx *ctx, const void *kern, size_t bytes) {
    static std::mutex mu;
    static std::map<std::pair<const void *, int>, size_t> granted;
    std::lock_guard<std::mutex> g(mu);
    size_t &have = granted[std::make_pair(kern, ctx->device)];
    if (bytes > have) {
        HIP_TRY(ctx, hipFuncSetAttribute(kern, hipFuncAttributeMaxDynamicSharedMemorySize, (int)bytes));
        have = bytes;
    }
    return ZIP_OK;
}

template <int E, bool HASH, int MODE = kStoreAll>
int32_t launch_commit(zip_ctx *ctx, const CommitArgs &a, uint32_t threads, uint32_t grid, hipStream_t st) {
    size_t lds = 512 + (size_t)E * (threads + 32 / E) * 12 + (size_t)a.row_len * 8 + 4 * kFinisherFlagWords;
    auto kern = raa_commit_kernel<E, HASH, MODE>;
    if (int32_t rc = ensure_dynamic_lds(ctx, reinterpret_cast<const void *>(kern), lds)) return rc;
    LaunchTimer t(ctx, HASH ? "raa_commit_kernel" : "raa_encode_kernel", st);
    hipLaunchKernelGGL(kern, dim3(grid), dim3(threads), lds, st, a);
    HIP_TRY(ctx, hipGetLastError());
    return ZIP_OK;
}

template <bool HASH, int MODE = kStoreAll>
int32_t launch_commit16(zip_ctx *ctx, const CommitArgs &a, uint32_t grid, hipStream_t st) {
    constexpr uint32_t T = 1024;
    auto kern = raa_commit16_kernel<T, HASH, MODE>;
    if (int32_t rc = ensure_dynamic_lds(ctx, reinterpret_cast<const void *>(kern), c16_lds_bytes(T))) return rc;
    LaunchTimer t(ctx, HASH ? "raa_commit_kernel" : "raa_encode_kernel", st);
    hipLaunchKernelGGL(kern, dim3(grid), dim3(T), c16_lds_bytes(T), st, a);
    HIP_TRY(ctx, hipGetLastError());
    return ZIP_OK;
}

template <bool HASH>
int32_t launch_commit_slab(zip_ctx *ctx, const CommitArgs &a, uint32_t grid, hipStream_t st) {
    auto kern = a.cw == 65536 ? raa_commit_slab_kernel<64, HASH> : raa_commit_slab_kernel<32, HASH>;
    if (int32_t rc = ensure_dynamic_lds(ctx, reinterpret_cast<const void *>(kern), cslab_lds_bytes())) return rc;
    LaunchTimer t(ctx, HASH ? "raa_commit_kernel" : "raa_encode_kernel", st);
    hipLaunchKernelGGL(kern, dim3(grid), dim3(kSlabThreads), cslab_lds_bytes(), st, a);
    HIP_TRY(ctx, hipGetLastError());
    return ZIP_OK;
}

struct CommitGeom {
    uint32_t e, threads;
    size_t lds;
};
CommitGeom commit_geom(uint32_t cw, uint32_t row_len) {
    CommitGeom g{};
    if (cw >= 32768) { g.e = cw / kSlabThreads; g.threads = kSlabThreads; g.lds = cslab_lds_bytes(); return g; }
    if (cw == 16384) { g.e = 16; g.threads = 1024; g.lds = c16_lds_bytes(1024); return g; }
    if (cw >= 512) { g.e = 8; g.threads = cw / 8; }
    else if (cw == 256) { g.e = 4; g.threads = 64; }
    else if (cw == 128) { g.e = 2; g.threads = 64; }
    else { g.e = 1; g.threads = 64; }
    g.lds = 512 + (size_t)g.e * (g.threads + 32 / g.e) * 12 + (size_t)row_len * 8 + 4 * kFinisherFlagWords;
    return g;
}
uint32_t commit_wgs_per_cu(const CommitGeom &g) {
    if (g.e > 16) return 1;
    uint32_t by_threads = 2048 / g.threads, by_lds = (uint32_t)((160u * 1024u) / g.lds);
    uint32_t k = by_threads < by_lds ? by_threads : by_lds;
    if (k > 8) k = 8;
    return k ? k : 1;
}

bool commit_supports_hint(uint32_t cw) { return cw >= 512 && cw <= 16384; }
constexpr uint32_t kRingSlots = 64, kRingChunks = 16, kRingStride = 16;
constexpr size_t kHintTables = 8192, kHintBytes = kHintTables + 8 * (8192 / 32) + 4 * 4096 + 64, kPackedRanksAt = kHintTables + 2048;
static bool packed_enabled() {
    return env_long("ZIP_HIP_PACKED", 1, 0, 1) != 0;
}
static void plan_packed(HintPlan &P) {
    const uint32_t cw = P.cw, wv = (cw + 31) / 32, w1 = (cw / 2 + 31) / 32;
    const uint32_t *sec[4] = {P.bm.data(), P.bm.data() + wv, P.bm.data() + 2 * wv, P.bm.data() + 2 * wv + w1};
    const uint32_t bits[4] = {cw, cw, cw / 2, cw / 4};
    const uint32_t waves = P.threads / 64, phases = P.e == 16 ? 2 : 1, sT = P.e == 16 ? 16 : P.threads;
    for (int k = 0; k < 4; k++) P.pos[k].assign(bits[k], 0xFFFF);
    P.wave_tab.assign((size_t)waves * phases * 16, 0);
    uint32_t cnt[4] = {0, 0, 0, 0};
    auto member = [&](int k, uint32_t i) { return (sec[k][i >> 5] >> (i & 31u)) & 1u; };
    for (uint32_t w = 0; w < waves; w++)
        for (uint32_t q = 0; q < phases; q++) {
            uint16_t base[32];
            auto stid = [&](uint32_t l) {
                const uint32_t tid = 64 * w + l;
                return P.e == 16 ? (tid & ~7u) * 16u + q * 8u + (tid & 7u) : tid;
            };
            auto site = [&](int k, int slot, uint32_t step, uint32_t shift, uint32_t cls, uint32_t ncls) {
                base[slot] = (uint16_t)cnt[k];
                for (uint32_t l = cls; l < 64; l += ncls) {
                    const uint32_t i = (step * sT + stid(l)) >> shift;
                    if (member(k, i)) P.pos[k][i] = (uint16_t)cnt[k]++;
                }
            };
            for (uint32_t e = 0; e < 8; e++) site(0, (int)e, e, 0, 0, 1);
            for (uint32_t e = 0; e < 8; e++) site(1, (int)(8 + e), e, 0, 0, 1);
            for (uint32_t g = 0; g < 4; g++)
                for (uint32_t par = 0; par < 2; par++) site(2, (int)(16 + 2 * g + par), 2 * g + par, 1, par, 2);
            for (uint32_t g = 0; g < 2; g++)
                for (uint32_t c4 = 0; c4 < 4; c4++) site(3, (int)(24 + 4 * g + c4), 4 * g + c4, 2, c4, 4);
            uint32_t *tab = P.wave_tab.data() + ((size_t)w * phases + q) * 16;
            for (uint32_t k = 0; k < 16; k++) tab[k] = (uint32_t)base[2 * k] | ((uint32_t)base[2 * k + 1] << 16);
        }
    uint32_t at = (cnt[0] * 16u + 127u) & ~127u;
    P.L.off[0] = at;
    at = (at + cnt[1] * 32u + 127u) & ~127u;
    P.L.off[1] = at;
    at = (at + cnt[2] * 32u + 127u) & ~127u;
    P.L.off[2] = at;
    at = (at + cnt[3] * 32u + 127u) & ~127u;
    P.L.stride = at;
}
static std::shared_ptr<HintPlan> get_hint_plan(zip_ctx *ctx, const uint32_t *cols, uint32_t n_cols, bool want_packed) {
    const uint32_t cw = ctx->p.codeword_len;
    const CommitGeom g = commit_geom(cw, ctx->p.row_len);
    if (ctx->hint_plan) {
        const HintPlan &h = *ctx->hint_plan;
        if (h.cw == cw && h.e == g.e && h.threads == g.threads && h.want_packed == want_packed && h.cols.size() == n_cols &&
            (n_cols == 0 || !memcmp(h.cols.data(), cols, (size_t)n_cols * 4)))
            return ctx->hint_plan;
    }
    auto P = std::make_shared<HintPlan>();
    P->cw = cw;
    P->e = g.e;
    P->threads = g.threads;
    P->want_packed = want_packed;
    P->cols.assign(cols, cols + n_cols);
    const uint32_t wv = (cw + 31) / 32, w1 = (cw / 2 + 31) / 32, w2 = (cw / 4 + 31) / 32;
    P->bm.assign(2 * (size_t)wv + w1 + w2, 0);
    uint32_t *nv = P->bm.data(), *n0 = nv + wv, *n1 = n0 + wv, *n2 = n1 + w1;
    for (uint32_t i = 0; i < n_cols; i++) {
        const uint32_t col = cols[i];
        nv[col >> 5] |= 1u << (col & 31);
        const uint32_t s0 = col ^ 1u, s1 = (col >> 1) ^ 1u, s2 = (col >> 2) ^ 1u;
        n0[s0 >> 5] |= 1u << (s0 & 31);
        n1[s1 >> 5] |= 1u << (s1 & 31);
        n2[s2 >> 5] |= 1u << (s2 & 31);
    }
    if (want_packed && n_cols && (g.e == 8 || g.e == 16) && cw >= 512 && g.threads % 64 == 0 && cw == g.e * g.threads &&
        ctx->depth >= 3) {
        plan_packed(*P);
        P->own_ranks.resize((size_t)n_cols * 4);
        P->packed = P->L.stride > 0 && P->wave_tab.size() * 4 <= kPackedRanksAt - kHintTables &&
                    kPackedRanksAt + P->own_ranks.size() * 2 <= kHintBytes && P->ranks(cols, n_cols, P->own_ranks.data());
    }
    std::vector<unsigned char> img(kHintBytes, 0);
    memcpy(img.data(), P->bm.data(), P->bm.size() * 4);
    size_t used = P->bm.size() * 4;
    if (P->packed) {
        memcpy(img.data() + kHintTables, P->wave_tab.data(), P->wave_tab.size() * 4);
        memcpy(img.data() + kPackedRanksAt, P->own_ranks.data(), P->own_ranks.size() * 2);
        used = kPackedRanksAt + P->own_ranks.size() * 2;
    }
    void *blk = nullptr;
    if (used <= kHintBytes && pool_alloc(ctx, kHintBytes, &blk) == ZIP_OK) {
        if (hipMemcpy(blk, img.data(), used, hipMemcpyHostToDevice) == hipSuccess) {
            P->dev = static_cast<unsigned char *>(blk);
            std::shared_ptr<bool> alive = ctx->alive;
            P->release = [ctx, alive](unsigned char *p) { if (*alive) pool_release(ctx, p); };
        } else {
            pool_release(ctx, blk);
            (void)hipGetLastError();
        }
    }
    ctx->hint_plan = P;
    return P;
}

template <bool HASH>
int32_t dispatch_commit(zip_ctx *ctx, CommitArgs a, uint32_t grid, hipStream_t st) {
    const CommitGeom g = commit_geom(a.cw, a.row_len);
    a.nact = a.cw / g.e < g.threads ? a.cw / g.e : g.threads;
    if (HASH && a.need) {
        if (g.e == 8 && a.pk) return launch_commit<8, HASH, HASH ? kStorePacked : kStoreAll>(ctx, a, g.threads, grid, st);
        if (g.e == 16 && a.pk) return launch_commit16<HASH, HASH ? kStorePacked : kStoreAll>(ctx, a, grid, st);
        a.pk = nullptr;
        if (g.e == 16) return launch_commit16<HASH, HASH ? kStoreHinted : kStoreAll>(ctx, a, grid, st);
        if (g.e == 8) return launch_commit<8, HASH, HASH ? kStoreHinted : kStoreAll>(ctx, a, g.threads, grid, st);
        a.need = nullptr;
    }
    a.pk = nullptr;
    switch (g.e) {
        case 64:
        case 32: return launch_commit_slab<HASH>(ctx, a, grid, st);
        case 16: return launch_commit16<HASH>(ctx, a, grid, st);
        case 8: return launch_commit<8, HASH>(ctx, a, g.threads, grid, st);
        case 4: return launch_commit<4, HASH>(ctx, a, g.threads, grid, st);
        case 2: return launch_commit<2, HASH>(ctx, a, g.threads, grid, st);
        default: return launch_commit<1, HASH>(ctx, a, g.threads, grid, st);
    }
}

template <int NL>
int32_t launch_upper(zip_ctx *ctx, hipStream_t st, uint32_t *layers, uint32_t *roots, uint32_t trees, uint32_t cw,
                     uint32_t level_in, uint32_t depth) {
    const uint64_t total = (uint64_t)trees * ((cw >> level_in) >> NL);
    const uint32_t threads = 256;
    const uint32_t blocks = (uint32_t)((total + threads - 1) / threads);
    LaunchTimer t(ctx, "merkle_upper_kernel", st);
    hipLaunchKernelGGL(merkle_upper_kernel<NL>, dim3(blocks), dim3(threads), 0, st, layers, roots, trees, cw,
                       level_in, depth);
    HIP_TRY(ctx, hipGetLastError());
    return ZIP_OK;
}

int32_t merkle_upper_levels(zip_ctx *ctx, hipStream_t st, uint32_t *layers, uint32_t *roots, uint32_t trees,
                            uint32_t cw, uint32_t level, uint32_t depth) {
    if (depth == 0) {
        LaunchTimer t(ctx, "copy_roots_depth0_kernel", st);
        hipLaunchKernelGGL(copy_roots_depth0_kernel, dim3((trees + 255) / 256), dim3(256), 0, st, layers, roots,
                           trees, cw);
        HIP_TRY(ctx, hipGetLastError());
        return ZIP_OK;
    }
    while (level < depth) {
        const uint32_t rem = depth - level;
        int32_t rc;
        if (rem >= 4) {
            rc = launch_upper<4>(ctx, st, layers, roots, trees, cw, level, depth);
            level += 4;
        } else if (rem == 3) {
            rc = launch_upper<3>(ctx, st, layers, roots, trees, cw, level, depth);
            level += 3;
        } else if (rem == 2) {
            rc = launch_upper<2>(ctx, st, layers, roots, trees, cw, level, depth);
            level += 2;
        } else {
            rc = launch_upper<1>(ctx, st, layers, roots, trees, cw, level, depth);
            level += 1;
        }
        if (rc) return rc;
    }
    return ZIP_OK;
}

int32_t stage_evals(zip_ctx *ctx, const int64_t *evals, zip_mem_kind kind, size_t n, Scratch &tmp,
                    const int64_t **dev) {
    if (!evals) return fail(ctx, ZIP_ERR_NULL, "evals is NULL");
    if (kind == ZIP_MEM_DEVICE) {
        *dev = evals;
        return ZIP_OK;
    }
    int32_t rc = tmp.get(n * 8);
    if (rc) return rc;
    if ((rc = copy_h2d_bounced(ctx, tmp.ptr, evals, n * 8, ctx->stream))) return rc;
    *dev = tmp.as<int64_t>();
    return ZIP_OK;
}

struct CombineOut {
    uint64_t *uprime = nullptr;
    uint64_t *row_limbs = nullptr;
    uint8_t *row_be = nullptr;
};

struct CombineScratch {
    Scratch pint, pa, pb;
    explicit CombineScratch(zip_ctx *c) : pint(c), pa(c), pb(c) {}
};

template <int FL>
int32_t run_combine_fl(zip_ctx *ctx, const int64_t *evals_d, const int64_t *coeffs_dv,
                       const uint64_t *q0_dv, const HostField *hf, bool do_int, bool do_field, const CombineOut &out,
                       CombineScratch *ext, int phase) {
    const uint32_t R = ctx->rows_local, C = ctx->p.row_len;
    const uint32_t bx = (C + 255) / 256;
    uint32_t chunks = 512 / bx;
    if (chunks > 32) chunks = 32;
    if (chunks < 1) chunks = 1;
    if (chunks > R) chunks = R;
    const uint32_t rpc = (R + chunks - 1) / chunks;
    chunks = (R + rpc - 1) / rpc;

    const hipStream_t st = ctx->stream;
    CombineScratch own(ctx);
    CombineScratch &cs = ext ? *ext : own;
    Scratch &pint = cs.pint, &pa = cs.pa, &pb = cs.pb;
    int32_t rc;
    CombineArgs a{};
    a.evals = evals_d;
    a.num_rows = R;
    a.row_len = C;
    a.rows_per_chunk = rpc;
    a.prio = 1;
    a.quirk_mod = hf ? hf->quirk_mod : 0;
    if (do_int) {
        if (phase != 2 && (rc = pint.get((size_t)chunks * C * 3 * 8))) return rc;
        a.coeffs = coeffs_dv;
        a.part_int = pint.as<uint64_t>();
    }
    if (do_field) {
        if (phase != 2 && (rc = pa.get((size_t)chunks * C * (FL + 2) * 8))) return rc;
        a.q0 = q0_dv;
        a.part_a = pa.as<uint64_t>();
    }
    if (phase != 2 && (rc = pb.get((size_t)chunks * (FL + 3) * 8))) return rc;
    a.part_k = pb.as<uint64_t>();
    if (phase != 2) {
        LaunchTimer t(ctx, "combine_rows_kernel", st);
        const dim3 grid(bx, chunks), block(256);
        if (a.quirk_mod && do_field) {
            if (do_int)
                hipLaunchKernelGGL((combine_rows_kernel<FL, true, true, true>), grid, block, 0, st, a);
            else
                hipLaunchKernelGGL((combine_rows_kernel<FL, false, true, true>), grid, block, 0, st, a);
// ... 985 lines not shown
            c->layers_bytes = (size_t)R * 2 * cw * 32;
            c->roots_bytes = (size_t)R * 32;
            if ((rc = pool_alloc(ctx, (size_t)((R + 3u) & ~3u) * 2 * cw * 32, (void **)&c->layers))) break;
            if ((rc = pool_alloc(ctx, c->roots_bytes, (void **)&c->roots))) break;
        }
        const int64_t *evals_d = evals;
        if (!evals) { rc = fail(ctx, ZIP_ERR_NULL, "evals is NULL"); break; }
        if (evals_kind == ZIP_MEM_HOST) {
            c->evals_bytes = n_evals * 8;
            if ((rc = pool_alloc(ctx, c->evals_bytes, (void **)&c->evals))) break;
            if ((rc = copy_h2d_bounced(ctx, c->evals, evals, c->evals_bytes, ctx->s_commit))) break;
            evals_d = c->evals;
        }
        const CommitGeom geom = commit_geom(cw, C);
        uint32_t G = ctx->num_cus * commit_wgs_per_cu(geom);
        if (G > R) G = R;
        const uint32_t rounds = (R + G - 1) / G;
        uint32_t nch = !with_merkle ? 1 : ctx->n_chunks ? ctx->n_chunks : rounds >= 8 ? std::min(8u, rounds / 4) : rounds >= 2 ? 2u : 1u;
        if (nch > rounds) nch = rounds;
        const uint32_t rpc = (rounds + nch - 1) / nch;
        nch = (rounds + rpc - 1) / rpc;
        std::vector<uint32_t> sched;
        if (with_merkle && rounds <= 64) {
            const char *env = ctx->knob_chunk_rounds.empty() ? nullptr : ctx->knob_chunk_rounds.c_str();
            if (env && !ctx->n_chunks) {
                uint32_t used = 0;
                for (const char *q = env; *q && used < rounds;) {
                    char *endp = nullptr;
                    const long v = strtol(q, &endp, 10);
                    if (endp == q) break;
                    if (v >= 1) {
                        const uint32_t take = std::min<uint32_t>((uint32_t)v, rounds - used);
                        sched.push_back(take);
                        used += take;
                    }
                    q = (*endp == ',') ? endp + 1 : endp;
                }
                if (!sched.empty() && used < rounds) sched.back() += rounds - used;
            }
            if (sched.empty() && !ctx->n_chunks && rounds >= 12) {
                const uint32_t n = rounds >= 24 ? std::min(kRingChunks, rounds / 2) : std::min(8u, rounds / 3), base = rounds / n;
                if (rounds >= 24 || base < 3) {
                    for (uint32_t k = 0; k + 1 < n; k++) sched.push_back(base);
                    sched.push_back(rounds - base * (n - 1));
                } else {
                    const uint32_t last = base * 2 / 3;
                    uint32_t extra = rounds - (base * (n - 1) + last);
                    for (uint32_t k = 0; k + 1 < n; k++) {
                        const uint32_t more = (extra + (n - 2 - k)) / (n - 1 - k);
                        sched.push_back(base + more);
                        extra -= more;
                    }
                    sched.push_back(last);
                }
            }
        }
        uint64_t chunk_ends = 0;
        if (sched.empty()) {
            for (uint32_t k = 0; k < nch; k++) sched.push_back(std::min(rpc, rounds - k * rpc));
        } else {
            nch = (uint32_t)sched.size();
            uint32_t r = 0;
            for (uint32_t k = 0; k < nch; k++) {
                r += sched[k];
                chunk_ends |= 1ull << (r - 1);
            }
        }
        c->bounds.resize(nch + 1);
        {
            uint64_t r = 0;
            for (uint32_t k = 0; k <= nch; k++) {
                const uint64_t b = r * G;
                c->bounds[k] = b < R ? (uint32_t)b : R;
                if (k < nch) r += sched[k];
            }
        }
        uint32_t classes = 1;
        {
            const long knob_classes = env_long("ZIP_HIP_CLASSES", 0, 1, 64);
            const uint32_t per_cu = commit_wgs_per_cu(geom);
            if (with_merkle && hint_cols && commit_supports_hint(cw) && rounds == 1 && R == G && per_cu >= 2 && G % 8 == 0 &&
                !ctx->n_chunks && knob_classes != 1) {
                classes = knob_classes > 1 ? (uint32_t)knob_classes : std::min(2u, per_cu);
                while (classes > 1 && ((G / 8) % classes || classes > per_cu)) classes--;
            }
            if (classes > 1) {
                nch = classes;
                chunk_ends = 0;
                c->bounds.resize(nch + 1);
                for (uint32_t k = 0; k <= nch; k++) c->bounds[k] = k * (G / classes);
            }
        }
        CommitArgs a{};
        a.classes = classes;
        a.evals = evals_d;
        a.perm1 = ctx->perm1_d;
        a.perm2 = ctx->perm2_d;
        a.rows = c->rows;
        a.compact_rows = c->compact_rows ? 1u : 0u;
        a.layers = c->layers;
        a.row_len = C;
        a.cw = cw;
        a.num_rows = R;
        a.rounds_per_chunk = rpc;
        a.chunk_ends = chunk_ends;
        a.roots = c->roots;
        a.clock = ctx->profiling ? ctx->clock_d : nullptr;
#ifdef ZIPK_DEBUG_STAMPS
        a.stamps = debug_stamps_buffer();
#endif
        hipError_t e = hipSuccess;
        if (with_merkle && hint_cols && commit_supports_hint(cw)) {
            const uint32_t wv = (cw + 31) / 32, w1 = (cw / 2 + 31) / 32, w2 = (cw / 4 + 31) / 32;
            const size_t words = 2 * (size_t)wv + w1 + w2;
            if (words * 4 > kHintBytes) { rc = fail(ctx, ZIP_ERR_UNSUPPORTED, "hint bitmaps exceed their staging block"); break; }
            const bool want_packed = c->compact_rows && n_hint && packed_enabled();
            c->plan = get_hint_plan(ctx, hint_cols, n_hint, want_packed);
            const bool resident = c->plan->dev != nullptr;
            if (!resident) {
                if (!ctx->hint_free.empty()) {
                    c->hint_h = ctx->hint_free.back();
                    ctx->hint_free.pop_back();
                } else if (hipHostMalloc((void **)&c->hint_h, kHintBytes, hipHostMallocDefault) != hipSuccess) {
                    c->hint_h = nullptr;
                    rc = fail(ctx, ZIP_ERR_ALLOC, "hipHostMalloc(%zu) failed", kHintBytes);
                    break;
                }
            }
            uint32_t *bm = resident ? nullptr : reinterpret_cast<uint32_t *>(c->hint_h);
            if (bm) memcpy(bm, c->plan->bm.data(), words * 4);
            const uint32_t *nv = c->plan->bm.data();
            c->hint_cols.assign(nv, nv + wv);
            size_t upload = words * 4;
            if (c->plan->packed) {
                if (!resident) {
                    memcpy(c->hint_h + kHintTables, c->plan->wave_tab.data(), c->plan->wave_tab.size() * 4);
                    memcpy(c->hint_h + kPackedRanksAt, c->plan->own_ranks.data(), c->plan->own_ranks.size() * 2);
                }
                upload = kPackedRanksAt + c->plan->own_ranks.size() * 2;
                c->packed = true;
                c->pk_stride = c->plan->L.stride;
                for (int k = 0; k < 3; k++) c->pk_off[k] = c->plan->L.off[k];
            }
            const unsigned char *tables_d;
            if (resident) {
                tables_d = c->plan->dev;
            } else {
                if ((rc = pool_alloc(ctx, kHintBytes, (void **)&c->need_d))) break;
                e = hipMemcpyAsync(c->need_d, bm, upload, hipMemcpyHostToDevice, ctx->s_commit);
                if (e != hipSuccess) { rc = fail(ctx, ZIP_ERR_HIP, "hint upload failed: %s", hipGetErrorString(e)); break; }
                tables_d = reinterpret_cast<const unsigned char *>(c->need_d);
            }
            a.need = reinterpret_cast<const uint32_t *>(tables_d);
            c->hinted = true;
            if (c->packed) {
                a.pk = reinterpret_cast<uint8_t *>(c->rows);
                a.pk_stride = c->pk_stride;
                a.pk_off0 = c->pk_off[0];
                a.pk_off1 = c->pk_off[1];
                a.pk_off2 = c->pk_off[2];
                a.pk_tab = reinterpret_cast<const uint32_t *>(tables_d + kHintTables);
                c->rank_d = reinterpret_cast<const uint16_t *>(tables_d + kPackedRanksAt);
            }
        }
        if (with_merkle && (nch > 1 || (hint_cols && R >= ctx->num_cus))) {
            if (nch <= kRingChunks && !ctx->ring_d) {
                if (hipMalloc((void **)&ctx->ring_d, (size_t)kRingSlots * kRingStride * 4) != hipSuccess ||
                    hipMemset(ctx->ring_d, 0, (size_t)kRingSlots * kRingStride * 4) != hipSuccess) {
                    if (ctx->ring_d) (void)hipFree(ctx->ring_d);
                    ctx->ring_d = nullptr;
                    (void)hipGetLastError();
                }
            }
            if (nch <= kRingChunks && ctx->ring_d) {
                if (ctx->ring_next == kRingSlots) {
                    if (e == hipSuccess) e = stream_wait(ctx->stream);
                    if (e == hipSuccess) e = stream_wait(ctx->s_commit);
                    if (e == hipSuccess) e = hipMemsetAsync(ctx->ring_d, 0, (size_t)kRingSlots * kRingStride * 4, ctx->s_commit);
                    if (e == hipSuccess) e = stream_wait(ctx->s_commit);
                    ctx->ring_next = 0;
                    ctx->ring_epoch++;
                }
                c->chunk_done = ctx->ring_d + (size_t)ctx->ring_next++ * kRingStride;
                c->ring_slot = true;
                c->ring_epoch = ctx->ring_epoch;
            } else {
                if ((rc = pool_alloc(ctx, (size_t)nch * 4, (void **)&c->chunk_done))) break;
                e = hipMemsetAsync(c->chunk_done, 0, (size_t)nch * 4, ctx->s_commit);
                c->zeroed = take_dep_event(ctx);
                if (e == hipSuccess) e = hipEventRecord(c->zeroed, ctx->s_commit);
            }
            a.chunk_done = c->chunk_done;
            c->expected.resize(nch);
            for (uint32_t k = 0; k < nch; k++) c->expected[k] = (R - c->bounds[k]) < G ? (R - c->bounds[k]) : G;
            if (classes > 1)
                for (uint32_t k = 0; k < nch; k++) c->expected[k] = G / classes;
        }
        if (e != hipSuccess) { rc = fail(ctx, ZIP_ERR_HIP, "commit setup failed: %s", hipGetErrorString(e)); break; }
        if (geom.e > 16) {
            const size_t need = (size_t)G * cw * 16;
            if (ctx->slab_bytes < need) {
                if (ctx->slab_d && (e = stream_wait(ctx->s_commit)) != hipSuccess) {
                    rc = fail(ctx, ZIP_ERR_HIP, "commit setup failed: %s", hipGetErrorString(e));
                    break;
                }
                if (ctx->slab_d) (void)hipFree(ctx->slab_d);
                ctx->slab_d = nullptr;
                ctx->slab_bytes = 0;
                if (hipMalloc((void **)&ctx->slab_d, need) != hipSuccess) {
                    ctx->slab_d = nullptr;
                    (void)hipGetLastError();
                    rc = fail(ctx, ZIP_ERR_ALLOC, "hipMalloc(%zu) of the commit slabs failed", need);
                    break;
                }
                ctx->slab_bytes = need;
            }
            a.slab = ctx->slab_d;
        }
        rc = with_merkle ? dispatch_commit<true>(ctx, a, G, ctx->s_commit) : dispatch_commit<false>(ctx, a, G, ctx->s_commit);
        if (rc) break;
        c->args = a;
        c->grid = G;
        c->evals_ref = evals_d;
        c->done = take_dep_event(ctx);
        e = hipEventRecord(c->done, ctx->s_commit);
        if (e != hipSuccess) rc = fail(ctx, ZIP_ERR_HIP, "commit pipeline failed: %s", hipGetErrorString(e));
        if (rc) break;
        if (with_merkle && roots_out) {
            if ((rc = wait_ready(c, ctx->stream))) break;
            if ((rc = deliver(ctx, roots_out, ZIP_MEM_HOST, c->roots, c->roots_bytes))) break;
        }
        if (evals_kind == ZIP_MEM_HOST) {
            hipError_t e = stream_wait(ctx->s_commit);
            if (e != hipSuccess) { rc = fail(ctx, ZIP_ERR_HIP, "commit failed: %s", hipGetErrorString(e)); break; }
        }
    } while (0);
    if (rc) {
        zip_commitment_free(c);
        return rc;
    }
    *out = c;
    return ZIP_OK;
}

static int32_t launch_witness_digest(zip_ctx *ctx, const int64_t *evals_d, size_t n, unsigned long long *out_d, hipStream_t st);

int32_t zip_commit(zip_ctx *ctx, const int64_t *evals, size_t n_evals, zip_mem_kind evals_kind,
                   int32_t with_merkle, uint8_t *roots_out, zip_commitment **out) {
    if (!ctx || !out) return ZIP_ERR_NULL;
    std::shared_ptr<HintPlan> plan;
    {
        std::lock_guard<std::recursive_mutex> api_lock(ctx->api_mu);
        if (with_merkle && (ctx->speculate == 2 || (ctx->speculate == 1 && evals_kind == ZIP_MEM_HOST)) && ctx->seen_columns &&
            ctx->hint_plan && ctx->hint_plan->cw == ctx->p.codeword_len &&
            !ctx->hint_plan->cols.empty() && commit_supports_hint(ctx->p.codeword_len))
            plan = ctx->hint_plan;
    }
    if (!plan) return commit_impl(ctx, evals, n_evals, evals_kind, with_merkle, nullptr, 0, roots_out, out);
    int32_t rc = commit_impl(ctx, evals, n_evals, evals_kind, 1, plan->cols.data(), (uint32_t)plan->cols.size(), roots_out, out);
    if (rc) return rc;
    zip_commitment *c = *out;
    std::lock_guard<std::recursive_mutex> api_lock(ctx->api_mu);
    c->speculative = true;
    if (c->hinted && !c->evals && c->evals_ref) {
        if (pool_alloc(ctx, 16, (void **)&c->digest_d) == ZIP_OK) {
            const size_t n = (size_t)ctx->rows_local * ctx->p.row_len;
            if (launch_witness_digest(ctx, c->evals_ref, n, c->digest_d, ctx->s_upper) == ZIP_OK) {
                c->digest_done = take_dep_event(ctx);
                (void)hipEventRecord(c->digest_done, ctx->s_upper);
            }
        }
    }
    return ZIP_OK;
}

int32_t zip_ctx_set_speculation(zip_ctx *ctx, int32_t on) {
    if (!ctx) return ZIP_ERR_NULL;
    std::lock_guard<std::recursive_mutex> api_lock(ctx->api_mu);
    ctx->speculate = on ? 2 : 0;
    return ZIP_OK;
}

int32_t zip_commit_hinted(zip_ctx *ctx, const int64_t *evals, size_t n_evals, zip_mem_kind evals_kind,
                          const uint32_t *cols, uint32_t n_cols, uint8_t *roots_out, zip_commitment **out) {
    if (!ctx || !out) return ZIP_ERR_NULL;
    if (n_cols && !cols) return ZIP_ERR_NULL;
    {
        std::lock_guard<std::recursive_mutex> api_lock(ctx->api_mu);
        if (int32_t rc = check_cols(ctx, cols, n_cols)) return rc;
    }
    static const uint32_t none = 0;
    return commit_impl(ctx, evals, n_evals, evals_kind, 1, cols ? cols : &none, n_cols, roots_out, out);
}

static int32_t launch_witness_digest(zip_ctx *ctx, const int64_t *evals_d, size_t n, unsigned long long *out_d, hipStream_t st) {
    HIP_TRY(ctx, hipMemsetAsync(out_d, 0, 16, st));
    const uint32_t blocks = (uint32_t)std::min<size_t>((n / 2 + 255) / 256, (size_t)ctx->num_cus);
    hipLaunchKernelGGL(witness_digest_kernel, dim3(blocks ? blocks : 1), dim3(256), 0, st, reinterpret_cast<const uint64_t *>(evals_d),
                       (uint64_t)n, out_d);
    HIP_TRY(ctx, hipGetLastError());
    return ZIP_OK;
}

static int32_t rematerialize(zip_commitment *c, const int64_t *evals_now = nullptr) {
    if (!c->hinted) return ZIP_OK;
    zip_ctx *ctx = c->ctx;
    CommitArgs a = c->args;
    a.need = nullptr;
    a.pk = nullptr;
    a.clock = nullptr;
    a.chunk_done = nullptr;
    a.evals = evals_now ? evals_now : c->evals ? c->evals : c->evals_ref;
    if (a.evals == c->evals_ref && !c->evals && c->speculative && c->digest_d) {
        const size_t n = (size_t)ctx->rows_local * ctx->p.row_len;
        Scratch again(ctx);
        int32_t rc = again.get(16);
        if (rc) return rc;
        if (c->digest_done) HIP_TRY(ctx, hipStreamWaitEvent(ctx->stream, c->digest_done, 0));
        if ((rc = launch_witness_digest(ctx, c->evals_ref, n, again.as<unsigned long long>(), ctx->stream))) return rc;
        unsigned long long then_[2] = {0, 0}, now_[2] = {1, 1};
        HIP_TRY(ctx, hipMemcpyAsync(then_, c->digest_d, 16, hipMemcpyDeviceToHost, ctx->stream));
        HIP_TRY(ctx, hipMemcpyAsync(now_, again.ptr, 16, hipMemcpyDeviceToHost, ctx->stream));
        HIP_TRY(ctx, stream_wait(ctx->stream));
        if (then_[0] != now_[0] || then_[1] != now_[1])
            return fail(ctx, ZIP_ERR_INVALID_PARAM,
                        "the device witness of this commitment has changed since zip_commit: the handle only holds what an "
                        "opening of the ctx's usual columns reads (speculative hint) and cannot be completed any more; keep the "
                        "witness until the handle is freed, or switch the speculation off (zip_ctx_set_speculation)");
    }
    if (c->done) HIP_TRY(ctx, hipStreamWaitEvent(ctx->s_commit, c->done, 0));
    HIP_TRY(ctx, stream_wait(ctx->stream));
    int32_t rc = dispatch_commit<true>(ctx, a, c->grid, ctx->s_commit);
    if (rc) return rc;
    if (c->done) HIP_TRY(ctx, hipEventRecord(c->done, ctx->s_commit));
    HIP_TRY(ctx, stream_wait(ctx->s_commit));
    c->hinted = false;
    c->packed = false;
    return ZIP_OK;
}

static int32_t ensure_columns(zip_commitment *c, const uint32_t *cols, uint32_t n_cols, const int64_t *evals_now = nullptr) {
    if (!c->hinted) return ZIP_OK;
    if (c->packed)
        return (c->plan && c->plan->cols.size() == n_cols && (n_cols == 0 || !memcmp(c->plan->cols.data(), cols, (size_t)n_cols * 4)))
                   ? ZIP_OK : rematerialize(c, evals_now);
    for (uint32_t i = 0; i < n_cols; i++) {
        const uint32_t col = cols[i];
        if ((col >> 5) >= c->hint_cols.size() || !((c->hint_cols[col >> 5] >> (col & 31)) & 1u)) return rematerialize(c, evals_now);
    }
    return ZIP_OK;
}

static void note_columns(zip_ctx *ctx, const uint32_t *cols, uint32_t n_cols) {
    if (!ctx->speculate || !n_cols || !commit_supports_hint(ctx->p.codeword_len)) return;
    (void)get_hint_plan(ctx, cols, n_cols, !ctx->no_compact && packed_enabled());
    ctx->seen_columns = true;
}

void zip_commitment_free(zip_commitment *c) {
    if (!c) return;
    std::lock_guard<std::recursive_mutex> api_lock(c->ctx->api_mu);
    if (c->done) {
        (void)event_wait(c->done);
        c->ctx->dep_event_pool.push_back(c->done);
    }
    if (c->zeroed) c->ctx->dep_event_pool.push_back(c->zeroed);
    for (hipEvent_t e : c->aux) c->ctx->dep_event_pool.push_back(e);
    if (c->ctx->stream && !c->consumers_done) (void)stream_wait(c->ctx->stream);
    if (!c->ring_slot) pool_release(c->ctx, c->chunk_done);
    if (c->digest_done) {
        (void)event_wait(c->digest_done);
        c->ctx->dep_event_pool.push_back(c->digest_done);
    }
    pool_release(c->ctx, c->digest_d);
    pool_release(c->ctx, c->need_d);
    if (c->hint_h) c->ctx->hint_free.push_back(c->hint_h);
    if (!c->borrows_rows) pool_release(c->ctx, c->rows);
    if (!c->borrows_rest) {
        pool_release(c->ctx, c->layers);
        pool_release(c->ctx, c->roots);
        pool_release(c->ctx, c->evals);
    }
    delete c;
}

static int32_t materialize_rows(zip_commitment *c);

int32_t zip_commitment_device_ptrs(zip_commitment *c, uint64_t **rows, uint8_t **layers, uint8_t **roots) {
    if (!c) return ZIP_ERR_NULL;
    std::lock_guard<std::recursive_mutex> api_lock(c->ctx->api_mu);
    int32_t rc_ = (rows || layers) ? rematerialize(c) : ZIP_OK;
    if (rc_) return rc_;
    if ((rc_ = wait_ready(c, c->ctx->stream))) return rc_;
    if (rows) {
        if ((rc_ = materialize_rows(c))) return rc_;
        *rows = c->rows;
    }
    if (layers) *layers = reinterpret_cast<uint8_t *>(c->layers);
    if (roots) *roots = reinterpret_cast<uint8_t *>(c->roots);
    return ZIP_OK;
}

static int32_t materialize_rows(zip_commitment *c) {
    if (!c->compact_rows) return ZIP_OK;
    zip_ctx *ctx = c->ctx;
    int32_t rc = wait_ready(c, ctx->stream);
    if (rc) return rc;
    const uint64_t n = c->rows_bytes / 16;
    void *full = nullptr;
    if ((rc = pool_alloc(ctx, (size_t)n * 32, &full))) return rc;
    const uint32_t blocks = (uint32_t)std::min<uint64_t>((n + 255) / 256, 65535);
    hipLaunchKernelGGL(expand_rows_kernel, dim3(blocks), dim3(256), 0, ctx->stream, reinterpret_cast<const uint4 *>(c->rows),
                       static_cast<uint4 *>(full), n);
    hipError_t e = hipGetLastError();
    if (e == hipSuccess) e = stream_wait(ctx->stream);
    if (e != hipSuccess) {
        (void)stream_wait(ctx->stream);
        pool_release(ctx, full);
        return fail(ctx, ZIP_ERR_HIP, "expanding the row entries failed: %s", hipGetErrorString(e));
    }
    if (!c->borrows_rows) pool_release(ctx, c->rows);
    c->borrows_rows = false;
    c->rows = static_cast<uint64_t *>(full);
    c->rows_bytes = (size_t)n * 32;
    c->compact_rows = false;
    return ZIP_OK;
}

int32_t zip_commit_download(zip_commitment *c, uint64_t *rows_out, uint8_t *layers_out, uint8_t *roots_out) {
    if (!c) return ZIP_ERR_NULL;
    zip_ctx *ctx = c->ctx;
    HIP_TRY(ctx, hipSetDevice(ctx->device));
    std::lock_guard<std::recursive_mutex> api_lock(ctx->api_mu);
    const uint32_t R = ctx->rows_local, cw = ctx->p.codeword_len;
    {
        int32_t rc_ = (rows_out || layers_out) ? rematerialize(c) : ZIP_OK;
        if (rc_) return rc_;
        if ((rc_ = wait_ready(c, ctx->stream))) return rc_;
    }
    if (rows_out) {
        int32_t rc_ = materialize_rows(c);
        if (rc_) return rc_;
        rc_ = copy_d2h_bounced(ctx, rows_out, c->rows, c->rows_bytes, ctx->stream);
        if (rc_) return rc_;
    }
    if (layers_out) {
        if (!c->layers) return fail(ctx, ZIP_ERR_INVALID_PARAM, "commitment has no Merkle trees (commit_no_merkle)");
        const size_t w = ((size_t)2 * cw - 2) * 32;
        if (w)
            HIP_TRY(ctx, hipMemcpy2DAsync(layers_out, w, c->layers, (size_t)2 * cw * 32, w, R, hipMemcpyDeviceToHost,
                                          ctx->stream));
    }
    if (roots_out) {
        if (!c->roots) return fail(ctx, ZIP_ERR_INVALID_PARAM, "commitment has no Merkle roots (commit_no_merkle)");
        HIP_TRY(ctx, hipMemcpyAsync(roots_out, c->roots, c->roots_bytes, hipMemcpyDeviceToHost, ctx->stream));
    }
    HIP_TRY(ctx, stream_wait(ctx->stream));
    return ZIP_OK;
}

int32_t zip_commitment_upload(zip_ctx *ctx, const uint64_t *rows, const uint8_t *layers, const uint8_t *roots,
// ... 1693 lines not shown
    c->have_second = true;
    return ZIP_OK;
}

int32_t zip_ccs_eval_matrices(zip_ccs *c, const uint64_t *r_x, const uint64_t *r_y, uint64_t *v_xy_out) {
    if (!c || !r_x || !r_y || !v_xy_out) return ZIP_ERR_NULL;
    zip_ctx *ctx = c->ctx;
    HIP_TRY(ctx, hipSetDevice(ctx->device));
    std::lock_guard<std::recursive_mutex> api_lock(ctx->api_mu);
    int32_t rc;
    if ((rc = zip_ccs_eq_table(c, r_x, 0))) return rc;
    if ((rc = zip_ccs_eq_table(c, r_y, 1))) return rc;
    c->have_second = false;
    HostField hf;
    if ((rc = ccs_field(c, &hf))) return rc;
    uint64_t *out_d = c->small_d + (size_t)33 * 8;
    CCS_DISPATCH_FL(c->fl, ccs_eval_matrices_fl, c, out_d, hf);
    if (rc) return rc;
    HIP_TRY(ctx, hipMemcpyAsync(v_xy_out, out_d, (size_t)c->t * c->fl * 8, hipMemcpyDeviceToHost, ctx->stream));
    HIP_TRY(ctx, stream_wait(ctx->stream));
    return ZIP_OK;
}

int32_t zip_ccs_table(zip_ccs *c, zip_ccs_table_kind which, uint32_t index, const uint64_t **table_dev) {
    if (!c || !table_dev) return ZIP_ERR_NULL;
    zip_ctx *ctx = c->ctx;
    *table_dev = nullptr;
    switch (which) {
        case ZIP_CCS_Z_FIELD:
            if (!c->have_z) return fail(ctx, ZIP_ERR_INVALID_PARAM, "zip_ccs_set_z has not run");
            *table_dev = c->z_f;
            return ZIP_OK;
        case ZIP_CCS_MZ:
            if (!c->have_z) return fail(ctx, ZIP_ERR_INVALID_PARAM, "zip_ccs_set_z has not run");
            if (index >= c->t) return fail(ctx, ZIP_ERR_INVALID_PARAM, "matrix %u of %u", index, c->t);
            *table_dev = c->mz[index];
            return ZIP_OK;
        case ZIP_CCS_EQ:
            if (index > 1 || !c->have_eq[index]) return fail(ctx, ZIP_ERR_INVALID_PARAM, "eq table %u has not been built", index);
            *table_dev = c->eq[index];
            return ZIP_OK;
        case ZIP_CCS_SECOND:
            if (!c->have_second) return fail(ctx, ZIP_ERR_INVALID_PARAM, "zip_ccs_second_table has not run");
            *table_dev = c->second;
            return ZIP_OK;
    }
    return fail(ctx, ZIP_ERR_INVALID_PARAM, "unknown table kind %d", (int)which);
}

int32_t zip_ccs_download(zip_ccs *c, zip_ccs_table_kind which, uint32_t index, uint64_t *out) {
    if (!c || !out) return ZIP_ERR_NULL;
    const uint64_t *d = nullptr;
    int32_t rc = zip_ccs_table(c, which, index, &d);
    if (rc) return rc;
    zip_ctx *ctx = c->ctx;
    HIP_TRY(ctx, hipSetDevice(ctx->device));
    return copy_d2h_bounced(ctx, out, d, (size_t)c->m * c->fl * 8, ctx->stream);
}

int32_t zip_sum_partials(zip_ctx *ctx, const uint64_t *uparts, const uint64_t *fparts, uint32_t n_parts,
                         const zip_field *field, uint64_t *uprime_out, uint64_t *row_out) {
    if (!ctx) return ZIP_ERR_NULL;
    HIP_TRY(ctx, hipSetDevice(ctx->device));
    std::lock_guard<std::recursive_mutex> api_lock(ctx->api_mu);
    if ((uparts && !uprime_out) || (fparts && !row_out)) return ZIP_ERR_NULL;
    HostField hf;
    hf.fl = 4;
    int32_t rc;
    if (fparts && (rc = make_field(ctx, field, &hf))) return rc;
    const uint32_t C = ctx->p.row_len;
    const dim3 grid((C + 255) / 256), block(256);
    LaunchTimer t(ctx, "sum_partials_kernel");
    switch (hf.fl) {
        case 2:
            hipLaunchKernelGGL(sum_partials_kernel<2>, grid, block, 0, ctx->stream, uparts, fparts, n_parts, C,
                               ctx->p.m_limbs, uprime_out, row_out, to_dev<2>(hf));
            break;
        case 3:
            hipLaunchKernelGGL(sum_partials_kernel<3>, grid, block, 0, ctx->stream, uparts, fparts, n_parts, C,
                               ctx->p.m_limbs, uprime_out, row_out, to_dev<3>(hf));
            break;
        default:
            hipLaunchKernelGGL(sum_partials_kernel<4>, grid, block, 0, ctx->stream, uparts, fparts, n_parts, C,
                               ctx->p.m_limbs, uprime_out, row_out, to_dev<4>(hf));
            break;
    }
    HIP_TRY(ctx, hipGetLastError());
    return ZIP_OK;
}

int32_t zip_merkle_trees(int32_t device, const uint64_t *leaves, uint32_t leaf_limbs, uint32_t depth,
                         uint32_t num_trees, zip_mem_kind kind, uint8_t *layers_out) {
    if (!leaves || !layers_out) return ZIP_ERR_NULL;
    if (leaf_limbs < 1 || leaf_limbs > 8 || depth > 24 || num_trees == 0) return ZIP_ERR_INVALID_PARAM;
    int ndev = 0;
    if (hipGetDeviceCount(&ndev) != hipSuccess || device < 0 || device >= ndev) return ZIP_ERR_NO_DEVICE;
    if (hipSetDevice(device) != hipSuccess) return ZIP_ERR_NO_DEVICE;
    zip_ctx *ctx = new (std::nothrow) zip_ctx();
    if (!ctx) return ZIP_ERR_ALLOC;
    ctx->device = device;
    int32_t rc = ZIP_OK;
    const uint32_t n = 1u << depth;
    const size_t leaf_bytes = (size_t)num_trees * n * leaf_limbs * 8;
    const size_t tree_bytes = (size_t)num_trees * 2 * n * 32;
    const size_t out_w = ((size_t)2 * n - 1) * 32;
    void *leaves_d = nullptr, *layers_d = nullptr, *roots_d = nullptr;
    do {
        if (hipStreamCreateWithFlags(&ctx->stream, hipStreamNonBlocking) != hipSuccess) { rc = ZIP_ERR_HIP; break; }
        if (kind == ZIP_MEM_HOST) {
            if ((rc = pool_alloc(ctx, leaf_bytes, &leaves_d))) break;
            if (hipMemcpyAsync(leaves_d, leaves, leaf_bytes, hipMemcpyHostToDevice, ctx->stream) != hipSuccess) { rc = ZIP_ERR_HIP; break; }
        } else {
            leaves_d = const_cast<uint64_t *>(leaves);
        }
        if ((rc = pool_alloc(ctx, tree_bytes, &layers_d))) break;
        if ((rc = pool_alloc(ctx, (size_t)num_trees * 32, &roots_d))) break;
        const size_t total = (size_t)num_trees * n;
        const dim3 grid((uint32_t)((total + 255) / 256)), block(256);
        const uint64_t *L = static_cast<const uint64_t *>(leaves_d);
        uint32_t *Y = static_cast<uint32_t *>(layers_d);
        switch (leaf_limbs) {
            case 1: hipLaunchKernelGGL(merkle_leaves_kernel<1>, grid, block, 0, ctx->stream, L, Y, num_trees, n); break;
            case 2: hipLaunchKernelGGL(merkle_leaves_kernel<2>, grid, block, 0, ctx->stream, L, Y, num_trees, n); break;
            case 3: hipLaunchKernelGGL(merkle_leaves_kernel<3>, grid, block, 0, ctx->stream, L, Y, num_trees, n); break;
            case 4: hipLaunchKernelGGL(merkle_leaves_kernel<4>, grid, block, 0, ctx->stream, L, Y, num_trees, n); break;
            case 5: hipLaunchKernelGGL(merkle_leaves_kernel<5>, grid, block, 0, ctx->stream, L, Y, num_trees, n); break;
            case 6: hipLaunchKernelGGL(merkle_leaves_kernel<6>, grid, block, 0, ctx->stream, L, Y, num_trees, n); break;
            case 7: hipLaunchKernelGGL(merkle_leaves_kernel<7>, grid, block, 0, ctx->stream, L, Y, num_trees, n); break;
            default: hipLaunchKernelGGL(merkle_leaves_kernel<8>, grid, block, 0, ctx->stream, L, Y, num_trees, n); break;
        }
        if (hipGetLastError() != hipSuccess) { rc = ZIP_ERR_HIP; break; }
        if ((rc = merkle_upper_levels(ctx, ctx->stream, Y, static_cast<uint32_t *>(roots_d), num_trees, n, 0, depth))) break;
        hipError_t e = hipMemcpy2DAsync(layers_out, out_w, layers_d, (size_t)2 * n * 32, out_w, num_trees,
                                        kind == ZIP_MEM_HOST ? hipMemcpyDeviceToHost : hipMemcpyDeviceToDevice,
                                        ctx->stream);
        if (e == hipSuccess) e = stream_wait(ctx->stream);
        if (e != hipSuccess) rc = ZIP_ERR_HIP;
    } while (0);
    if (kind != ZIP_MEM_HOST) {
        std::lock_guard<std::mutex> g(ctx->mu);
        ctx->live_blocks.erase(leaves_d);
    }
    zip_ctx_destroy(ctx);
    return rc;
}

int32_t zip_ctx_set_profiling(zip_ctx *ctx, int32_t on) {
    if (!ctx) return ZIP_ERR_NULL;
    ctx->profiling = on != 0;
    ctx->profile_commit_only = on == 2;
    return ZIP_OK;
}

int32_t zip_ctx_commit_clock(zip_ctx *ctx, double *mhz_out) {
    if (!ctx || !mhz_out) return ZIP_ERR_NULL;
    HIP_TRY(ctx, hipSetDevice(ctx->device));
    std::lock_guard<std::recursive_mutex> api_lock(ctx->api_mu);
    if (ctx->s_commit) HIP_TRY(ctx, stream_wait(ctx->s_commit));
    const unsigned long long *c = ctx->clock_h;
    *mhz_out = (c && c[3] > c[1] && c[2] > c[0]) ? (double)(c[2] - c[0]) / (double)(c[3] - c[1]) * 100.0 : 0.0;
    return ZIP_OK;
}

int32_t zip_ctx_profile_read(zip_ctx *ctx, zip_kernel_time *out, uint32_t cap) {
    if (!ctx) return ZIP_ERR_NULL;
    HIP_TRY(ctx, hipSetDevice(ctx->device));
    std::lock_guard<std::recursive_mutex> api_lock(ctx->api_mu);
    HIP_TRY(ctx, stream_wait(ctx->stream));
    for (auto &pe : ctx->pending) {
        float ms = 0.f;
        if (hipEventElapsedTime(&ms, pe.start, pe.stop) == hipSuccess) {
            KernelStat &s = ctx->stats[pe.name];
            s.launches++;
            s.total_ms += ms;
        }
        ctx->event_pool.push_back(pe.start);
        ctx->event_pool.push_back(pe.stop);
    }
    ctx->pending.clear();
    ctx->stat_names.clear();
    ctx->stat_names.reserve(ctx->stats.size());
    uint32_t n = 0;
    for (auto &kv : ctx->stats) {
        ctx->stat_names.push_back(kv.first);
        if (out && n < cap) {
            out[n].name = ctx->stat_names.back().c_str();
            out[n].launches = kv.second.launches;
            out[n].total_ms = kv.second.total_ms;
        }
        n++;
    }
    ctx->stats.clear();
    return (int32_t)n;
}

}
```

Baseline: 11190.

## Use 96-bit asm carry arithmetic in scans and precompute store masks on host

Replaces the i128-based prefix sums and the block-wide exclusive scan with a three-word i96 type driven by inline assembly: carry-chained adds and DPP row_shr/row_bcast steps, plus a smaller 16-byte LDS slot for wave totals. Separately, the per-thread store masks used by masked commits are now computed once on the host in the hint plan, placed in the resident hint table, and read by the kernel instead of being rebuilt from the need bitmaps every launch. A C ABI entry is also exported for computing these masks. The aim is to cut wide-integer ALU work and bitmap gathers, at the cost of hand-scheduled asm with manual s_nop hazards that can break on other targets, and a larger hint block.

```diff
diff --git a/include/zip_hip.h b/include/zip_hip.h
--- a/include/zip_hip.h
+++ b/include/zip_hip.h
@@ -211,6 +211,8 @@
     float total_ms;
 } zip_kernel_time;
 int32_t zip_ctx_set_profiling(zip_ctx *ctx, int32_t on);
+int32_t zip_hint_store_masks(uint32_t entries_per_thread, uint32_t codeword_len, uint32_t threads, const uint32_t *need,
+                             uint32_t *out);
 int32_t zip_ctx_commit_clock(zip_ctx *ctx, double *mhz_out);
 int32_t zip_ctx_profile_read(zip_ctx *ctx, zip_kernel_time *out, uint32_t cap);
 
diff --git a/zinc_amd/cabi.py b/zinc_amd/cabi.py
--- a/zinc_amd/cabi.py
+++ b/zinc_amd/cabi.py
@@ -21,7 +21,7 @@
     "zip_ctx_last_error", "zip_ctx_synchronize", "zip_ctx_stream", "zip_ctx_set_speculation", "zip_commit", "zip_commit_hinted", "zip_commit_open", "zip_commit_open_begin", "zip_job_wait", "zip_commitment_free",
     "zip_commitment_device_ptrs", "zip_commit_download", "zip_commitment_upload", "zip_open_testing",
     "zip_open_columns", "zip_open_eval", "zip_proof_len", "zip_open", "zip_open_shard", "zip_sum_partials", "zip_merkle_trees",
-    "zip_ctx_set_profiling", "zip_ctx_profile_read", "zip_ctx_commit_clock",
+    "zip_ctx_set_profiling", "zip_ctx_profile_read", "zip_ctx_commit_clock", "zip_hint_store_masks",
     "zip_mctx_create", "zip_mctx_destroy", "zip_mctx_last_error", "zip_mctx_shards", "zip_mctx_shard_ctx", "zip_mctx_set_witness",
     "zip_mctx_commit_open", "zip_mctx_shard_openings", "zip_mctx_ends", "zip_mctx_roots", "zip_mctx_roots_path", "zip_verify", "zip_mle_eval", "zip_commitment_mle_eval", "zip_field_map_int256",
     "zip_open_stream", "zip_sumcheck_init", "zip_sumcheck_round", "zip_sumcheck_round_begin", "zip_sumcheck_round_end", "zip_sumcheck_last_error", "zip_sumcheck_free",
@@ -245,6 +245,9 @@
     L.zip_ctx_profile_read.argtypes = [vp, C.POINTER(KernelTime), C.c_uint32]
     L.zip_ctx_commit_clock.argtypes = [vp, C.POINTER(C.c_double)]
     L.zip_ctx_commit_clock.restype = C.c_int32
+    if hasattr(L, "zip_hint_store_masks"):
+        L.zip_hint_store_masks.argtypes = [C.c_uint32, C.c_uint32, C.c_uint32, u32p, u32p]
+        L.zip_hint_store_masks.restype = C.c_int32
     L.zip_mctx_create.argtypes = [C.POINTER(ZipParams), C.c_int32, C.POINTER(C.c_int32), C.POINTER(vp)]
     L.zip_mctx_destroy.argtypes = [vp]
     L.zip_mctx_destroy.restype = None
diff --git a/zinc_amd/csrc/kernels_commit.cuh b/zinc_amd/csrc/kernels_commit.cuh
--- a/zinc_amd/csrc/kernels_commit.cuh
+++ b/zinc_amd/csrc/kernels_commit.cuh
@@ -3,6 +3,7 @@
 #include <stdint.h>
 
 #include "blake3.cuh"
+#include "store_mask.h"
 
 namespace zipk {
 
@@ -37,6 +38,7 @@
     uint32_t *chunk_done;
     uint32_t classes;
     const uint32_t *need;
+    const uint32_t *smask;
     unsigned long long *clock;
     uint4 *slab;
 #ifdef ZIPK_DEBUG_STAMPS
@@ -44,56 +46,188 @@
 #endif
 };
 
-__device__ __forceinline__ i128 shfl_up_i96(i128 x, int off) {
-    uint32_t d0 = (uint32_t)x, d1 = (uint32_t)((u128)x >> 32), d2 = (uint32_t)((u128)x >> 64);
-    d0 = __shfl_up(d0, off, 64);
-    d1 = __shfl_up(d1, off, 64);
-    d2 = __shfl_up(d2, off, 64);
-    const int64_t hi = (int64_t)(int32_t)d2;
-    return (i128)(((u128)(uint64_t)hi << 64) | ((u128)d1 << 32) | d0);
-}
-
 __device__ __forceinline__ void lds_barrier() {
     asm volatile("s_waitcnt lgkmcnt(0)\n\ts_barrier" ::: "memory");
 }
 
-template <int CTRL, int ROW_MASK>
-__device__ __forceinline__ i128 dpp_i96(i128 x) {
-    const int d0 = (int)(uint32_t)x, d1 = (int)(uint32_t)((u128)x >> 32), d2 = (int)(uint32_t)((u128)x >> 64);
-    const uint32_t y0 = (uint32_t)__builtin_amdgcn_update_dpp(0, d0, CTRL, ROW_MASK, 0xF, false);
-    const uint32_t y1 = (uint32_t)__builtin_amdgcn_update_dpp(0, d1, CTRL, ROW_MASK, 0xF, false);
-    const uint32_t y2 = (uint32_t)__builtin_amdgcn_update_dpp(0, d2, CTRL, ROW_MASK, 0xF, false);
-    const int64_t hi = (int64_t)(int32_t)y2;
-    return (i128)(((u128)(uint64_t)hi << 64) | ((u128)y1 << 32) | y0);
-}
-
-__device__ __forceinline__ i128 block_exclusive_scan_i96(i128 total, i128 *wave_tot, int which) {
-    const int lane = threadIdx.x & 63;
+#define ZIPK_SCAN_I96 1
+struct i96 {
+    uint32_t w0, w1, w2;
+};
+__device__ __forceinline__ i96 i96_zero() { return i96{0u, 0u, 0u}; }
+__device__ __forceinline__ i96 i96_from_i64(int64_t x) {
+    return i96{(uint32_t)(uint64_t)x, (uint32_t)((uint64_t)x >> 32), (uint32_t)(int32_t)(x >> 63)};
+}
+__device__ __forceinline__ i96 i96_from_parts(uint64_t lo, uint32_t hi) { return i96{(uint32_t)lo, (uint32_t)(lo >> 32), hi}; }
+__device__ __forceinline__ uint64_t i96_lo64(const i96 &x) { return (uint64_t)x.w0 | ((uint64_t)x.w1 << 32); }
+__device__ __forceinline__ i96 i96_from_i128(i128 x) {
+    return i96{(uint32_t)x, (uint32_t)((u128)x >> 32), (uint32_t)((u128)x >> 64)};
+}
+__device__ __forceinline__ i128 i96_to_i128(const i96 &x) {
+    return (i128)(((u128)(uint64_t)(int64_t)(int32_t)x.w2 << 64) | ((u128)x.w1 << 32) | x.w0);
+}
+
+__device__ __forceinline__ void i96_add1(i96 &a, const i96 &p) {
+    asm("v_add_co_u32_e32 %0, vcc, %3, %0\n\t"
+        "s_nop 1\n\t"
+        "v_addc_co_u32_e32 %1, vcc, %4, %1, vcc\n\t"
+        "s_nop 1\n\t"
+        "v_addc_co_u32_e32 %2, vcc, %5, %2, vcc"
+        : "+v"(a.w0), "+v"(a.w1), "+v"(a.w2)
+        : "v"(p.w0), "v"(p.w1), "v"(p.w2)
+        : "vcc");
+}
+__device__ __forceinline__ void i96_add1_s(i96 &a, uint32_t p0, uint32_t p1, uint32_t p2) {
+    uint32_t t1, t2;
+    asm("s_nop 1\n\t"
+        "v_add_co_u32_e32 %0, vcc, %5, %0\n\t"
+        "v_mov_b32_e32 %3, %6\n\t"
+        "v_mov_b32_e32 %4, %7\n\t"
+        "v_addc_co_u32_e32 %1, vcc, %3, %1, vcc\n\t"
+        "s_nop 1\n\t"
+        "v_addc_co_u32_e32 %2, vcc, %4, %2, vcc"
+        : "+v"(a.w0), "+v"(a.w1), "+v"(a.w2), "=&v"(t1), "=&v"(t2)
+        : "s"(p0), "s"(p1), "s"(p2)
+        : "vcc");
+}
+#define ZIPK_I96_LO(d, c, s) "v_add_co_u32_e64 " d ", " c ", " d ", " s "\n\t"
+#define ZIPK_I96_HI(d, c, s) "v_addc_co_u32_e64 " d ", " c ", " d ", " s ", " c "\n\t"
+__device__ __forceinline__ void i96_add3(i96 &a, i96 &b, i96 &c, const i96 &p) {
+    uint64_t c0, c1, c2;
+    asm(ZIPK_I96_LO("%0", "%9", "%12") ZIPK_I96_LO("%3", "%10", "%12") ZIPK_I96_LO("%6", "%11", "%12")
+        ZIPK_I96_HI("%1", "%9", "%13") ZIPK_I96_HI("%4", "%10", "%13") ZIPK_I96_HI("%7", "%11", "%13")
+        ZIPK_I96_HI("%2", "%9", "%14") ZIPK_I96_HI("%5", "%10", "%14") ZIPK_I96_HI("%8", "%11", "%14")
+        : "+v"(a.w0), "+v"(a.w1), "+v"(a.w2), "+v"(b.w0), "+v"(b.w1), "+v"(b.w2), "+v"(c.w0), "+v"(c.w1), "+v"(c.w2),
+          "=&s"(c0), "=&s"(c1), "=&s"(c2)
+        : "v"(p.w0), "v"(p.w1), "v"(p.w2));
+}
+__device__ __forceinline__ void i96_add2(i96 &a, i96 &b, const i96 &p) {
+    uint64_t c0, c1;
+    asm(ZIPK_I96_LO("%0", "%6", "%8") ZIPK_I96_LO("%3", "%7", "%8") "s_nop 0\n\t"
+        ZIPK_I96_HI("%1", "%6", "%9") ZIPK_I96_HI("%4", "%7", "%9") "s_nop 0\n\t"
+        ZIPK_I96_HI("%2", "%6", "%10") ZIPK_I96_HI("%5", "%7", "%10")
+        : "+v"(a.w0), "+v"(a.w1), "+v"(a.w2), "+v"(b.w0), "+v"(b.w1), "+v"(b.w2), "=&s"(c0), "=&s"(c1)
+        : "v"(p.w0), "v"(p.w1), "v"(p.w2));
+}
+__device__ __forceinline__ void i96_prefix3(i96 &a, i96 &b, i96 &c, const i96 &p) {
+    uint64_t c0, c1, c2;
+    asm(ZIPK_I96_LO("%0", "%9", "%12") ZIPK_I96_LO("%3", "%10", "%0") ZIPK_I96_LO("%6", "%11", "%3")
+        ZIPK_I96_HI("%1", "%9", "%13") ZIPK_I96_HI("%4", "%10", "%1") ZIPK_I96_HI("%7", "%11", "%4")
+        ZIPK_I96_HI("%2", "%9", "%14") ZIPK_I96_HI("%5", "%10", "%2") ZIPK_I96_HI("%8", "%11", "%5")
+        : "+v"(a.w0), "+v"(a.w1), "+v"(a.w2), "+v"(b.w0), "+v"(b.w1), "+v"(b.w2), "+v"(c.w0), "+v"(c.w1), "+v"(c.w2),
+          "=&s"(c0), "=&s"(c1), "=&s"(c2)
+        : "v"(p.w0), "v"(p.w1), "v"(p.w2));
+}
+__device__ __forceinline__ void i96_prefix2(i96 &a, i96 &b, const i96 &p) {
+    uint64_t c0, c1;
+    asm(ZIPK_I96_LO("%0", "%6", "%8") ZIPK_I96_LO("%3", "%7", "%0") "s_nop 0\n\t"
+        ZIPK_I96_HI("%1", "%6", "%9") ZIPK_I96_HI("%4", "%7", "%1") "s_nop 0\n\t"
+        ZIPK_I96_HI("%2", "%6", "%10") ZIPK_I96_HI("%5", "%7", "%2")
+        : "+v"(a.w0), "+v"(a.w1), "+v"(a.w2), "+v"(b.w0), "+v"(b.w1), "+v"(b.w2), "=&s"(c0), "=&s"(c1)
+        : "v"(p.w0), "v"(p.w1), "v"(p.w2));
+}
+#undef ZIPK_I96_LO
+#undef ZIPK_I96_HI
+
+template <int E, int E0 = 1>
+__device__ __forceinline__ void i96_prefix(i96 (&v)[E]) {
+    if constexpr (E - E0 >= 3) {
+        i96_prefix3(v[E0], v[E0 + 1], v[E0 + 2], v[E0 - 1]);
+        i96_prefix<E, E0 + 3>(v);
+    } else if constexpr (E - E0 == 2) {
+        i96_prefix2(v[E0], v[E0 + 1], v[E0 - 1]);
+    } else if constexpr (E - E0 == 1) {
+        i96_add1(v[E0], v[E0 - 1]);
+    }
+}
+template <int E, int E0 = 0>
+__device__ __forceinline__ void i96_add_all(i96 (&v)[E], const i96 &p) {
+    if constexpr (E - E0 >= 3) {
+        i96_add3(v[E0], v[E0 + 1], v[E0 + 2], p);
+        i96_add_all<E, E0 + 3>(v, p);
+    } else if constexpr (E - E0 == 2) {
+        i96_add2(v[E0], v[E0 + 1], p);
+    } else if constexpr (E - E0 == 1) {
+        i96_add1(v[E0], p);
+    }
+}
+
+struct __align__(16) i96_slot {
+    uint32_t w0, w1, w2, unused;
+};
+
+#define ZIPK_DPP_FULL " row_mask:0xf bank_mask:0xf bound_ctrl:0\n\t"
+#define ZIPK_SCAN_STEP(ctrl, fill_a, fill_b)                              \
+    "v_add_co_u32_dpp %0, vcc, %0, %0 " ctrl ZIPK_DPP_FULL fill_a         \
+    "v_addc_co_u32_dpp %1, vcc, %1, %1, vcc " ctrl ZIPK_DPP_FULL fill_b   \
+    "v_addc_co_u32_dpp %2, vcc, %2, %2, vcc " ctrl ZIPK_DPP_FULL
+#define ZIPK_SCAN_BCAST(ctrl, mask)                                       \
+    "v_mov_b32_dpp %3, %0 " ctrl " row_mask:" mask " bank_mask:0xf\n\t"  \
+    "v_mov_b32_dpp %4, %1 " ctrl " row_mask:" mask " bank_mask:0xf\n\t"  \
+    "v_mov_b32_dpp %5, %2 " ctrl " row_mask:" mask " bank_mask:0xf\n\t"  \
+    "v_add_co_u32_e32 %0, vcc, %3, %0\n\t"                                \
+    "v_mov_b32_e32 %3, 0\n\t"                                             \
+    "s_nop 0\n\t"                                                         \
+    "v_addc_co_u32_e32 %1, vcc, %4, %1, vcc\n\t"                          \
+    "v_mov_b32_e32 %4, 0\n\t"                                             \
+    "s_nop 0\n\t"                                                         \
+    "v_addc_co_u32_e32 %2, vcc, %5, %2, vcc\n\t"                          \
+    "v_mov_b32_e32 %5, 0\n\t"
+
+__device__ __forceinline__ i96 block_exclusive_scan_i96(const i96 &total, i96_slot *wave_tot, int which) {
+    int lane = threadIdx.x & 63;
+    asm volatile("" : "+v"(lane));
     const int wid = __builtin_amdgcn_readfirstlane((int)(threadIdx.x >> 6));
-    i128 x = total;
-    x += dpp_i96<0x111, 0xF>(x);
-    x += dpp_i96<0x112, 0xF>(x);
-    x += dpp_i96<0x114, 0xF>(x);
-    x += dpp_i96<0x118, 0xF>(x);
-    x += dpp_i96<0x142, 0xA>(x);
-    x += dpp_i96<0x143, 0xC>(x);
-    i128 *tot = wave_tot + 16 * which;
-    if (lane == 63) tot[wid] = x;
+    uint32_t x0 = total.w0, x1 = total.w1, x2 = total.w2;
+    uint32_t t0, t1, t2;
+    asm volatile("s_nop 1\n\t"
+        ZIPK_SCAN_STEP("row_shr:1", "s_nop 1\n\t", "s_nop 1\n\t")
+        ZIPK_SCAN_STEP("row_shr:2", "s_nop 1\n\t", "s_nop 1\n\t")
+        ZIPK_SCAN_STEP("row_shr:4", "s_nop 1\n\t", "s_nop 1\n\t")
+        ZIPK_SCAN_STEP("row_shr:8", "v_mov_b32_e32 %3, 0\n\tv_mov_b32_e32 %4, 0\n\t", "v_mov_b32_e32 %5, 0\n\ts_nop 0\n\t")
+        "s_nop 1\n\t"
+        ZIPK_SCAN_BCAST("row_bcast:15", "0xa")
+        "s_nop 0\n\t"
+        ZIPK_SCAN_BCAST("row_bcast:31", "0xc")
+        "v_mov_b32_dpp %3, %0 wave_shr:1" ZIPK_DPP_FULL
+        "v_mov_b32_dpp %4, %1 wave_shr:1" ZIPK_DPP_FULL
+        "v_mov_b32_dpp %5, %2 wave_shr:1" ZIPK_DPP_FULL
+        "s_nop 0"
+        : "+v"(x0), "+v"(x1), "+v"(x2), "=&v"(t0), "=&v"(t1), "=&v"(t2)
+        :
+        : "vcc");
+    i96_slot *tot = wave_tot + 16 * which;
+    if (lane == 63) {
+        tot[wid].w0 = x0;
+        tot[wid].w1 = x1;
+        tot[wid].w2 = x2;
+    }
     lds_barrier();
-    i128 t = lane < 16 ? tot[lane] : (i128)0;
-    t += dpp_i96<0x111, 0xF>(t);
-    t += dpp_i96<0x112, 0xF>(t);
-    t += dpp_i96<0x114, 0xF>(t);
-    t += dpp_i96<0x118, 0xF>(t);
-    i128 base = 0;
-    if (wid > 0) {
-        const uint32_t b0 = (uint32_t)__builtin_amdgcn_readlane((int)(uint32_t)t, wid - 1);
-        const uint32_t b1 = (uint32_t)__builtin_amdgcn_readlane((int)(uint32_t)((u128)t >> 32), wid - 1);
-        const uint32_t b2 = (uint32_t)__builtin_amdgcn_readlane((int)(uint32_t)((u128)t >> 64), wid - 1);
-        base = (i128)(((u128)(uint64_t)(int64_t)(int32_t)b2 << 64) | ((u128)b1 << 32) | b0);
-    }
-    return base + (x - total);
-}
+    uint32_t s0 = 0, s1 = 0, s2 = 0;
+    if (lane >= 1 && lane < 16) {
+        s0 = tot[lane - 1].w0;
+        s1 = tot[lane - 1].w1;
+        s2 = tot[lane - 1].w2;
+    }
+    asm volatile("s_nop 1\n\t"
+        ZIPK_SCAN_STEP("row_shr:1", "s_nop 1\n\t", "s_nop 1\n\t")
+        ZIPK_SCAN_STEP("row_shr:2", "s_nop 1\n\t", "s_nop 1\n\t")
+        ZIPK_SCAN_STEP("row_shr:4", "s_nop 1\n\t", "s_nop 1\n\t")
+        ZIPK_SCAN_STEP("row_shr:8", "s_nop 1\n\t", "s_nop 1\n\t")
+        "s_nop 0"
+        : "+v"(s0), "+v"(s1), "+v"(s2)
+        :
+        : "vcc");
+    const uint32_t b0 = (uint32_t)__builtin_amdgcn_readlane((int)s0, wid);
+    const uint32_t b1 = (uint32_t)__builtin_amdgcn_readlane((int)s1, wid);
+    const uint32_t b2 = (uint32_t)__builtin_amdgcn_readlane((int)s2, wid);
+    i96 pre{t0, t1, t2};
+    i96_add1_s(pre, b0, b1, b2);
+    return pre;
+}
+#undef ZIPK_SCAN_STEP
+#undef ZIPK_SCAN_BCAST
+#undef ZIPK_DPP_FULL
 
 __device__ __forceinline__ void store_hash(uint32_t *dst, const uint32_t (&h)[8]) {
     uint4 *d = reinterpret_cast<uint4 *>(dst);
@@ -246,29 +380,6 @@
     }
 };
 
-template <int E>
-__device__ __forceinline__ uint32_t store_mask(const uint32_t *need, uint32_t cw, uint32_t base, uint32_t T, uint32_t tid) {
-    if (!need) return 0xFFFFFFFFu;
-    const uint32_t *nv = need, *n0 = nv + (cw + 31) / 32, *n1 = n0 + (cw + 31) / 32, *n2 = n1 + (cw / 2 + 31) / 32;
-    uint32_t m = 0;
-#pragma unroll
-    for (int e = 0; e < E; e++) {
-        const uint32_t j = base + e * T + tid;
-        m |= ((nv[j >> 5] >> (j & 31)) & 1u) << e;
-        m |= ((n0[j >> 5] >> (j & 31)) & 1u) << (8 + e);
-    }
-#pragma unroll
-    for (int g = 0; g < E / 2; g++) {
-        const uint32_t i = (base + (2 * g + (tid & 1u)) * T + tid) >> 1;
-        m |= ((n1[i >> 5] >> (i & 31)) & 1u) << (16 + g);
-    }
-#pragma unroll
-    for (int g = 0; g < E / 4; g++) {
-        const uint32_t i = (base + (4 * g + (tid & 3u)) * T + tid) >> 2;
-        m |= ((n2[i >> 5] >> (i & 31)) & 1u) << (24 + g);
-    }
-    return m;
-}
 
 template <int E, int E0, class Src>
 __device__ __forceinline__ void store_rows_only(Src &src) {
@@ -551,7 +662,7 @@
     const bool active = tid0 < a.nact;
     stamp_clock(a, 0);
 
-    i128 *wave_tot = reinterpret_cast<i128 *>(smem);
+    i96_slot *wave_tot = reinterpret_cast<i96_slot *>(smem);
     uint64_t *t2lo = reinterpret_cast<uint64_t *>(smem + 512);
     uint32_t *t2hi = reinterpret_cast<uint32_t *>(t2lo + E * PS);
     int64_t *rowbuf = reinterpret_cast<int64_t *>(t2hi + E * PS);
@@ -569,7 +680,7 @@
         }
     };
     load_pidx(tid0);
-    const uint32_t smask = (MASKED && active) ? store_mask<E>(a.need, cw, 0u, a.nact, tid0) : 0xFFFFFFFFu;
+    const uint32_t smask = !(MASKED && active) ? 0xFFFFFFFFu : a.smask ? a.smask[tid0] : store_mask<E>(a.need, cw, 0u, a.nact, tid0);
     uint32_t ptab[16] = {};
     if (MODE == kStorePacked) {
         const uint32_t *wt = a.pk_tab + (size_t)__builtin_amdgcn_readfirstlane(tid0 >> 6) * 16;
@@ -624,25 +735,24 @@
             for (int k = 0; k < NPF; k++) nxt[k] = nin[k * T + tid];
         }
 
-        i128 v[E];
+        i96 v[E];
         if (active) {
 #pragma unroll
-            for (int e = 0; e < E; e++) v[e] = (i128)rowbuf[(pidx[e] ^ z) & 0xFFFFu];
-#pragma unroll
-            for (int e = 1; e < E; e++) v[e] += v[e - 1];
+            for (int e = 0; e < E; e++) v[e] = i96_from_i64(rowbuf[(pidx[e] ^ z) & 0xFFFFu]);
+            i96_prefix<E>(v);
         } else {
 #pragma unroll
-            for (int e = 0; e < E; e++) v[e] = 0;
+            for (int e = 0; e < E; e++) v[e] = i96_zero();
         }
         {
-            const i128 pre = block_exclusive_scan_i96(v[E - 1], wave_tot, 0);
+            const i96 pre = block_exclusive_scan_i96(v[E - 1], wave_tot, 0);
             if (active) {
+                i96_add_all<E>(v, pre);
 #pragma unroll
                 for (int e = 0; e < E; e++) {
-                    v[e] += pre;
                     const uint32_t slot = e * PS + tid;
-                    t2lo[slot] = (uint64_t)v[e];
-                    t2hi[slot] = (uint32_t)((u128)v[e] >> 64);
+                    t2lo[slot] = i96_lo64(v[e]);
+                    t2hi[slot] = v[e].w2;
                 }
             }
         }
@@ -651,25 +761,21 @@
 #pragma unroll
             for (int e = 0; e < E; e++) {
                 const uint32_t slot = (pidx[e] ^ z) >> 16;
-                const uint64_t lo = t2lo[slot];
-                const int64_t hi = (int64_t)(int32_t)t2hi[slot];
-                v[e] = (i128)(((u128)(uint64_t)hi << 64) | lo);
-            }
-#pragma unroll
-            for (int e = 1; e < E; e++) v[e] += v[e - 1];
+                v[e] = i96_from_parts(t2lo[slot], t2hi[slot]);
+            }
+            i96_prefix<E>(v);
         }
         {
-            const i128 pre = block_exclusive_scan_i96(v[E - 1], wave_tot, 1);
-#pragma unroll
-            for (int e = 0; e < E; e++) v[e] += pre;
+            const i96 pre = block_exclusive_scan_i96(v[E - 1], wave_tot, 1);
+            i96_add_all<E>(v, pre);
         }
 
         if (active) {
 #pragma unroll
             for (int e = 0; e < E; e++) {
                 const uint32_t slot = e * PS + tid;
-                t2lo[slot] = (uint64_t)v[e];
-                t2hi[slot] = (uint32_t)((u128)v[e] >> 64);
+                t2lo[slot] = i96_lo64(v[e]);
+                t2hi[slot] = v[e].w2;
             }
         }
         if (prefetch && has_next) {
@@ -761,15 +867,21 @@
     const uint32_t cw = a.cw, row_len = a.row_len;
     stamp_clock(a, 0);
 
-    i128 *wave_tot = reinterpret_cast<i128 *>(smem);
+    i96_slot *wave_tot = reinterpret_cast<i96_slot *>(smem);
     uint64_t *t2lo = reinterpret_cast<uint64_t *>(smem + 512);
     int8_t *t2dh = reinterpret_cast<int8_t *>(t2lo + (size_t)E * PS);
     int32_t *ghi = reinterpret_cast<int32_t *>(t2dh + (size_t)E * PS);
     uint64_t *park_lo = reinterpret_cast<uint64_t *>(smem + 512);
     uint32_t *park_hi = reinterpret_cast<uint32_t *>(park_lo + (size_t)8 * PS);
 
-    const uint32_t smask0 = MASKED ? store_mask<8>(a.need, cw, 0u, 16u, (tid0 & ~7u) * 16u + (tid0 & 7u)) : 0xFFFFFFFFu;
-    const uint32_t smask1 = MASKED ? store_mask<8>(a.need, cw, 0u, 16u, (tid0 & ~7u) * 16u + 8u + (tid0 & 7u)) : 0xFFFFFFFFu;
+    uint32_t smask0 = 0xFFFFFFFFu, smask1 = 0xFFFFFFFFu;
+    if (MASKED && a.smask) {
+        smask0 = a.smask[tid0];
+        smask1 = a.smask[T + tid0];
+    } else if (MASKED) {
+        smask0 = store_mask<8>(a.need, cw, 0u, 16u, store_mask16_tid(tid0, 0u));
+        smask1 = store_mask<8>(a.need, cw, 0u, 16u, store_mask16_tid(tid0, 1u));
+    }
     uint32_t ptab0[16] = {}, ptab1[16] = {};
     if (MODE == kStorePacked) {
         const uint32_t *wt = a.pk_tab + (size_t)__builtin_amdgcn_readfirstlane(tid0 >> 6) * 32;
@@ -793,34 +905,33 @@
         uint64_t *out_row = a.rows + (size_t)row * cw * (a.compact_rows ? 2 : 4);
 
         uint32_t p2[E];
-        i128 v[E];
+        i96 v[E];
         {
             const uint4 *q1 = reinterpret_cast<const uint4 *>(a.perm1 + (size_t)tid * E);
             const uint4 *q2 = reinterpret_cast<const uint4 *>(a.perm2 + (size_t)tid * E);
 #pragma unroll
             for (int k = 0; k < E / 4; k++) {
                 const uint4 s1 = q1[k], s2 = q2[k];
-                v[4 * k + 0] = (i128)in[s1.x & (row_len - 1)];
-                v[4 * k + 1] = (i128)in[s1.y & (row_len - 1)];
-                v[4 * k + 2] = (i128)in[s1.z & (row_len - 1)];
-                v[4 * k + 3] = (i128)in[s1.w & (row_len - 1)];
+                v[4 * k + 0] = i96_from_i64(in[s1.x & (row_len - 1)]);
+                v[4 * k + 1] = i96_from_i64(in[s1.y & (row_len - 1)]);
+                v[4 * k + 2] = i96_from_i64(in[s1.z & (row_len - 1)]);
+                v[4 * k + 3] = i96_from_i64(in[s1.w & (row_len - 1)]);
                 p2[4 * k + 0] = s2.x;
                 p2[4 * k + 1] = s2.y;
                 p2[4 * k + 2] = s2.z;
                 p2[4 * k + 3] = s2.w;
             }
         }
-#pragma unroll
-        for (int e = 1; e < E; e++) v[e] += v[e - 1];
+        i96_prefix<E>(v);
         {
-            const i128 pre = block_exclusive_scan_i96(v[E - 1], wave_tot, 0);
-            const int32_t phi = (int32_t)(uint32_t)((u128)pre >> 64);
+            const i96 pre = block_exclusive_scan_i96(v[E - 1], wave_tot, 0);
+            const int32_t phi = (int32_t)pre.w2;
             ghi[tid] = phi;
+            i96_add_all<E>(v, pre);
 #pragma unroll
             for (int e = 0; e < E; e++) {
-                const i128 t = v[e] + pre;
-                t2lo[e * PS + tid] = (uint64_t)t;
-                t2dh[e * PS + tid] = (int8_t)((int32_t)(uint32_t)((u128)t >> 64) - phi);
+                t2lo[e * PS + tid] = i96_lo64(v[e]);
+                t2dh[e * PS + tid] = (int8_t)((int32_t)v[e].w2 - phi);
             }
         }
         lds_barrier();
@@ -828,28 +939,24 @@
         for (int e = 0; e < E; e++) {
             const uint32_t j = p2[e];
             const uint32_t slot = (j & 15u) * PS + (j >> 4);
-            const uint64_t lo = t2lo[slot];
-            const int64_t hi = (int64_t)(ghi[j >> 4] + (int32_t)t2dh[slot]);
-            v[e] = (i128)(((u128)(uint64_t)hi << 64) | lo);
-        }
-#pragma unroll
-        for (int e = 1; e < E; e++) v[e] += v[e - 1];
+            v[e] = i96_from_parts(t2lo[slot], (uint32_t)(ghi[j >> 4] + (int32_t)t2dh[slot]));
+        }
+        i96_prefix<E>(v);
         {
-            const i128 pre = block_exclusive_scan_i96(v[E - 1], wave_tot, 1);
-#pragma unroll
-            for (int e = 0; e < E; e++) v[e] += pre;
+            const i96 pre = block_exclusive_scan_i96(v[E - 1], wave_tot, 1);
+            i96_add_all<E>(v, pre);
         }
 #pragma unroll
         for (int e = 8; e < E; e++) {
-            park_lo[(e - 8) * PS + tid] = (uint64_t)v[e];
-            park_hi[(e - 8) * PS + tid] = (uint32_t)((u128)v[e] >> 64);
+            park_lo[(e - 8) * PS + tid] = i96_lo64(v[e]);
+            park_hi[(e - 8) * PS + tid] = v[e].w2;
         }
         uint32_t x0[8], x1[8], x2[8];
 #pragma unroll
         for (int e = 0; e < 8; e++) {
-            x0[e] = (uint32_t)(uint64_t)v[e];
-            x1[e] = (uint32_t)((uint64_t)v[e] >> 32);
-            x2[e] = (uint32_t)((u128)v[e] >> 64);
+            x0[e] = v[e].w0;
+            x1[e] = v[e].w1;
+            x2[e] = v[e].w2;
         }
 #pragma unroll
         for (uint32_t q = 0; q < 2; q++) {
@@ -927,7 +1034,7 @@
     const uint32_t cw = a.cw, row_len = a.row_len;
     stamp_clock(a, 0);
 
-    i128 *wave_tot = reinterpret_cast<i128 *>(smem);
+    i96_slot *wave_tot = reinterpret_cast<i96_slot *>(smem);
     i128 *pre1 = reinterpret_cast<i128 *>(smem + 512);
     i128 *runp = pre1 + T;
     uint4 *slab = a.slab + (size_t)blockIdx.x * cw;
@@ -958,7 +1065,7 @@
                 }
             }
         }
-        pre1[tid] = block_exclusive_scan_i96(s, wave_tot, 0);
+        pre1[tid] = i96_to_i128(block_exclusive_scan_i96(i96_from_i128(s), wave_tot, 0));
         vmem_barrier();
 
         const uint4 *q2 = reinterpret_cast<const uint4 *>(a.perm2 + (size_t)tid * E);
@@ -973,7 +1080,7 @@
                 s += slab_get(slab[(size_t)(j & (E - 1)) * T + (j >> LOGE)]) + pre1[j >> LOGE];
             }
         }
-        runp[tid] = block_exclusive_scan_i96(s, wave_tot, 1);
+        runp[tid] = i96_to_i128(block_exclusive_scan_i96(i96_from_i128(s), wave_tot, 1));
 
 #pragma unroll 1
         for (uint32_t q = 0; q < (uint32_t)E / 8u; q++) {
diff --git a/zinc_amd/csrc/store_mask.h b/zinc_amd/csrc/store_mask.h
--- /dev/null
+++ b/zinc_amd/csrc/store_mask.h
@@ -0,0 +1,38 @@
+#pragma once
+#include <stdint.h>
+
+#if defined(__HIPCC__)
+#define ZIPK_HOST_DEVICE __host__ __device__ __forceinline__
+#else
+#define ZIPK_HOST_DEVICE inline
+#endif
+
+namespace zipk {
+
+template <int E>
+ZIPK_HOST_DEVICE uint32_t store_mask(const uint32_t *need, uint32_t cw, uint32_t base, uint32_t T, uint32_t tid) {
+    if (!need) return 0xFFFFFFFFu;
+    const uint32_t *nv = need, *n0 = nv + (cw + 31) / 32, *n1 = n0 + (cw + 31) / 32, *n2 = n1 + (cw / 2 + 31) / 32;
+    uint32_t m = 0;
+#pragma unroll
+    for (int e = 0; e < E; e++) {
+        const uint32_t j = base + e * T + tid;
+        m |= ((nv[j >> 5] >> (j & 31)) & 1u) << e;
+        m |= ((n0[j >> 5] >> (j & 31)) & 1u) << (8 + e);
+    }
+#pragma unroll
+    for (int g = 0; g < E / 2; g++) {
+        const uint32_t i = (base + (2 * g + (tid & 1u)) * T + tid) >> 1;
+        m |= ((n1[i >> 5] >> (i & 31)) & 1u) << (16 + g);
+    }
+#pragma unroll
+    for (int g = 0; g < E / 4; g++) {
+        const uint32_t i = (base + (4 * g + (tid & 3u)) * T + tid) >> 2;
+        m |= ((n2[i >> 5] >> (i & 31)) & 1u) << (24 + g);
+    }
+    return m;
+}
+
+ZIPK_HOST_DEVICE uint32_t store_mask16_tid(uint32_t t, uint32_t q) { return (t & ~7u) * 16u + q * 8u + (t & 7u); }
+
+}
diff --git a/zinc_amd/csrc/zip_hip.hip b/zinc_amd/csrc/zip_hip.hip
--- a/zinc_amd/csrc/zip_hip.hip
+++ b/zinc_amd/csrc/zip_hip.hip
@@ -70,6 +70,7 @@
     std::vector<uint32_t> wave_tab;
     std::vector<uint16_t> pos[4];
     std::vector<uint16_t> own_ranks;
+    std::vector<uint32_t> smask;
     unsigned char *dev = nullptr;
     std::function<void(unsigned char *)> release;
     HintPlan() = default;
@@ -801,7 +802,28 @@
 
 bool commit_supports_hint(uint32_t cw) { return cw >= 512 && cw <= 16384; }
 constexpr uint32_t kRingSlots = 64, kRingChunks = 16, kRingStride = 16;
-constexpr size_t kHintTables = 8192, kHintBytes = kHintTables + 8 * (8192 / 32) + 4 * 4096 + 64, kPackedRanksAt = kHintTables + 2048;
+constexpr size_t kHintTables = 8192, kPackedRanksAt = kHintTables + 2048;
+constexpr size_t kStoreMasksAt = kHintTables + 8 * (8192 / 32) + 4 * 4096 + 64;
+constexpr size_t kHintBytes = kStoreMasksAt + 2 * 1024 * 4;
+static bool plan_masks_enabled() {
+    return env_long("ZIP_HIP_PLAN_MASKS", 1, 0, 1) != 0;
+}
+static size_t plan_store_masks(uint32_t e, uint32_t cw, uint32_t threads, const uint32_t *need, uint32_t *out) {
+    for (uint32_t t = 0; t < threads; t++) {
+        switch (e) {
+            case 1: out[t] = zipk::store_mask<1>(need, cw, 0u, threads, t); break;
+            case 2: out[t] = zipk::store_mask<2>(need, cw, 0u, threads, t); break;
+            case 4: out[t] = zipk::store_mask<4>(need, cw, 0u, threads, t); break;
+            case 8: out[t] = zipk::store_mask<8>(need, cw, 0u, threads, t); break;
+            case 16:
+                out[t] = zipk::store_mask<8>(need, cw, 0u, 16u, zipk::store_mask16_tid(t, 0u));
+                out[threads + t] = zipk::store_mask<8>(need, cw, 0u, 16u, zipk::store_mask16_tid(t, 1u));
+                break;
+            default: return 0;
+        }
+    }
+    return (size_t)threads * (e == 16 ? 2 : 1);
+}
 static bool packed_enabled() {
     return env_long("ZIP_HIP_PACKED", 1, 0, 1) != 0;
 }
@@ -879,6 +901,10 @@
         P->packed = P->L.stride > 0 && P->wave_tab.size() * 4 <= kPackedRanksAt - kHintTables &&
                     kPackedRanksAt + P->own_ranks.size() * 2 <= kHintBytes && P->ranks(cols, n_cols, P->own_ranks.data());
     }
+    if (commit_supports_hint(cw) && (g.e == 8 || g.e == 16) && cw == g.e * g.threads && g.threads <= 1024) {
+        P->smask.resize((size_t)g.threads * (g.e == 16 ? 2 : 1));
+        if (!plan_store_masks(g.e, cw, g.threads, P->bm.data(), P->smask.data())) P->smask.clear();
+    }
     std::vector<unsigned char> img(kHintBytes, 0);
     memcpy(img.data(), P->bm.data(), P->bm.size() * 4);
     size_t used = P->bm.size() * 4;
@@ -886,6 +912,10 @@
         memcpy(img.data() + kHintTables, P->wave_tab.data(), P->wave_tab.size() * 4);
         memcpy(img.data() + kPackedRanksAt, P->own_ranks.data(), P->own_ranks.size() * 2);
         used = kPackedRanksAt + P->own_ranks.size() * 2;
+    }
+    if (!P->smask.empty()) {
+        memcpy(img.data() + kStoreMasksAt, P->smask.data(), P->smask.size() * 4);
+        used = kStoreMasksAt + P->smask.size() * 4;
     }
     void *blk = nullptr;
     if (used <= kHintBytes && pool_alloc(ctx, kHintBytes, &blk) == ZIP_OK) {
@@ -2177,6 +2207,8 @@
                 tables_d = reinterpret_cast<const unsigned char *>(c->need_d);
             }
             a.need = reinterpret_cast<const uint32_t *>(tables_d);
+            if (resident && !c->plan->smask.empty() && plan_masks_enabled())
+                a.smask = reinterpret_cast<const uint32_t *>(tables_d + kStoreMasksAt);
             c->hinted = true;
             if (c->packed) {
                 a.pk = reinterpret_cast<uint8_t *>(c->rows);
@@ -2332,6 +2364,7 @@
     zip_ctx *ctx = c->ctx;
     CommitArgs a = c->args;
     a.need = nullptr;
+    a.smask = nullptr;
     a.pk = nullptr;
     a.clock = nullptr;
     a.chunk_done = nullptr;
@@ -4331,6 +4364,13 @@
     return ZIP_OK;
 }
 
+int32_t zip_hint_store_masks(uint32_t entries_per_thread, uint32_t codeword_len, uint32_t threads, const uint32_t *need,
+                             uint32_t *out) {
+    if (!need || !out) return ZIP_ERR_NULL;
+    if (!threads || threads > 1024 || (uint64_t)entries_per_thread * threads != codeword_len) return ZIP_ERR_INVALID_PARAM;
+    return plan_store_masks(entries_per_thread, codeword_len, threads, need, out) ? ZIP_OK : ZIP_ERR_INVALID_PARAM;
+}
+
 int32_t zip_ctx_commit_clock(zip_ctx *ctx, double *mhz_out) {
     if (!ctx || !mhz_out) return ZIP_ERR_NULL;
     HIP_TRY(ctx, hipSetDevice(ctx->device));
```

Result: no change. 11170 (-0.2%).
